# HeyWeCome/WhisprRec

Measured on AMD Instinct MI355X. Metric: BPR training triplets/sec, higher is better.
Workload: dtype f32; 1 GPU; BPRMF emb_size=64, synthetic 1000000 users x 1000000 items (uniform ids), batch 65536, SGD l2=0, plan build in timed region; batch=65536, emb_size=64, optimizer=SGD, plan_chunk_batches=64, tables=single GPU, step_stream=whisprrec_amd.hip_ops.PipelinedSgd, plan=group plan (no per-batch sort: flags + lists of the shared rows, wr_group.hip), chained_step_launch=True, plan_build=on a side stream, beside the steps of the chunk before

## Files before the change

### include/whisprrec_hip.h

```cpp
#ifndef WHISPRREC_HIP_H
#define WHISPRREC_HIP_H

#include <stdint.h>

#ifdef __cplusplus
extern "C" {
#endif

#define WR_ABI_VERSION 1

#define WR_OK 0
#define WR_E_NULL (-1)
#define WR_E_SHAPE (-2)
#define WR_E_WORKSPACE (-3)
#define WR_E_ALIGN (-4)
#define WR_E_RANGE (-5)

int32_t wr_abi_version(void);
const char *wr_last_error(void);
int32_t wr_device_info(int32_t *n_cu, int32_t *wave_size, char *arch, int32_t arch_len);

int64_t wr_bpr_fwd_workspace_bytes(int64_t B);
int32_t wr_bpr_fwd(const float *user_tab, int64_t n_users, const float *item_tab, int64_t n_items, int32_t D,
                   const int64_t *u, const int64_t *p, const int64_t *n, int64_t B, float *pos_score, float *neg_score,
                   float *coef, float *loss, void *workspace, int64_t workspace_bytes, void *stream);

int64_t wr_bprmf_plan_workspace_bytes(int64_t n_triplets, int64_t batch_size, int64_t n_users, int64_t n_items);
int32_t wr_bprmf_plan_build_i64(const int64_t *u, const int64_t *p, const int64_t *n, int64_t n_triplets,
                                int64_t batch_size, int64_t n_users, int64_t n_items, int32_t *tu, int32_t *tp,
                                int32_t *tn, int32_t *torig, int32_t *oc_item, int32_t *oc_src, int32_t *err_flag,
                                void *workspace, int64_t workspace_bytes, void *stream);
int32_t wr_bprmf_plan_build_i32(const int32_t *u, const int32_t *p, const int32_t *n, int64_t n_triplets,
                                int64_t batch_size, int64_t n_users, int64_t n_items, int32_t *tu, int32_t *tp,
                                int32_t *tn, int32_t *torig, int32_t *oc_item, int32_t *oc_src, int32_t *err_flag,
                                void *workspace, int64_t workspace_bytes, void *stream);

int64_t wr_bprmf_plan_small_max_batch(void);
int32_t wr_bprmf_plan_build_small_i64(const int64_t *u, const int64_t *p, const int64_t *n, int64_t n_triplets,
                                      int64_t batch_size, int64_t n_users, int64_t n_items, int32_t *tu, int32_t *tp,
                                      int32_t *tn, int32_t *torig, int32_t *oc_item, int32_t *oc_src, int32_t *err_flag,
                                      void *stream);
int32_t wr_bprmf_plan_build_small_i32(const int32_t *u, const int32_t *p, const int32_t *n, int64_t n_triplets,
                                      int64_t batch_size, int64_t n_users, int64_t n_items, int32_t *tu, int32_t *tp,
                                      int32_t *tn, int32_t *torig, int32_t *oc_item, int32_t *oc_src, int32_t *err_flag,
                                      void *stream);

int64_t wr_bprmf_plan_fast_workspace_bytes(int64_t n_triplets, int64_t batch_size, int64_t n_users, int64_t n_items);
int32_t wr_bprmf_plan_build_fast_i64(const int64_t *u, const int64_t *p, const int64_t *n, int64_t n_triplets,
                                     int64_t batch_size, int64_t n_users, int64_t n_items, int32_t *tu, int32_t *tp,
                                     int32_t *tn, int32_t *torig, int32_t *oc_item, int32_t *oc_src, int32_t *flags,
                                     void *workspace, int64_t workspace_bytes, void *stream);
int32_t wr_bprmf_plan_build_fast_i32(const int32_t *u, const int32_t *p, const int32_t *n, int64_t n_triplets,
                                     int64_t batch_size, int64_t n_users, int64_t n_items, int32_t *tu, int32_t *tp,
                                     int32_t *tn, int32_t *torig, int32_t *oc_item, int32_t *oc_src, int32_t *flags,
                                     void *workspace, int64_t workspace_bytes, void *stream);

int32_t wr_bprmf_plan_fast_marks_supported(int64_t n_triplets, int64_t batch_size, int64_t n_users, int64_t n_items);
int32_t wr_bprmf_plan_build_fast_marks_i64(const int64_t *u, const int64_t *p, const int64_t *n, int64_t n_triplets,
                                           int64_t batch_size, int64_t n_users, int64_t n_items, int32_t *tu, int32_t *tp,
                                           int32_t *tn, int32_t *torig, int32_t *oc_item, int32_t *oc_src, int32_t *flags,
                                           void *workspace, int64_t workspace_bytes, int32_t *bitmap, void *stream);
int32_t wr_bprmf_plan_build_fast_marks_i32(const int32_t *u, const int32_t *p, const int32_t *n, int64_t n_triplets,
                                           int64_t batch_size, int64_t n_users, int64_t n_items, int32_t *tu, int32_t *tp,
                                           int32_t *tn, int32_t *torig, int32_t *oc_item, int32_t *oc_src, int32_t *flags,
                                           void *workspace, int64_t workspace_bytes, int32_t *bitmap, void *stream);

typedef struct wr_bucket_side {
    int32_t n_buckets;
    const int32_t *row_bucket;
    const int32_t *bucket_start;
    const int32_t *bucket_rows;
    const int32_t *bucket_sub;
} wr_bucket_side;

int64_t wr_bprmf_plan_fast_mapped_workspace_bytes(int64_t n_triplets, int64_t batch_size, int64_t n_users, int64_t n_items,
                                                  int32_t n_buckets_users, int32_t n_buckets_items);
int32_t wr_bprmf_plan_build_fast_mapped_i64(const int64_t *u, const int64_t *p, const int64_t *n, int64_t n_triplets,
                                            int64_t batch_size, int64_t n_users, int64_t n_items,
                                            const wr_bucket_side *map_users, const wr_bucket_side *map_items, int32_t *tu,
                                            int32_t *tp, int32_t *tn, int32_t *torig, int32_t *oc_item, int32_t *oc_src,
                                            int32_t *flags, void *workspace, int64_t workspace_bytes, void *stream);
int32_t wr_bprmf_plan_build_fast_mapped_i32(const int32_t *u, const int32_t *p, const int32_t *n, int64_t n_triplets,
                                            int64_t batch_size, int64_t n_users, int64_t n_items,
                                            const wr_bucket_side *map_users, const wr_bucket_side *map_items, int32_t *tu,
                                            int32_t *tp, int32_t *tn, int32_t *torig, int32_t *oc_item, int32_t *oc_src,
                                            int32_t *flags, void *workspace, int64_t workspace_bytes, void *stream);

int32_t wr_sample_negatives_i64(const int64_t *users, int64_t n, int64_t n_users, int64_t n_items, const int64_t *clicked_ptr,
                                const int32_t *clicked_idx, uint64_t seed, uint64_t epoch, int64_t *neg_items,
                                int32_t *err_flag, void *stream);
int32_t wr_sample_negatives_i32(const int32_t *users, int64_t n, int64_t n_users, int64_t n_items, const int64_t *clicked_ptr,
                                const int32_t *clicked_idx, uint64_t seed, uint64_t epoch, int32_t *neg_items,
                                int32_t *err_flag, void *stream);

int32_t wr_epoch_prepare_range_i64(const int64_t *users, const int64_t *items, int64_t n, int64_t n_users, int64_t n_items,
                                   const int64_t *clicked_ptr, const int32_t *clicked_idx, uint64_t seed, uint64_t epoch,
                                   int64_t first, int64_t count, int64_t *out_users, int64_t *out_pos, int64_t *out_neg,
                                   int64_t *order_out, int32_t *err_flag, void *stream);
int32_t wr_epoch_prepare_range_i32(const int32_t *users, const int32_t *items, int64_t n, int64_t n_users, int64_t n_items,
                                   const int64_t *clicked_ptr, const int32_t *clicked_idx, uint64_t seed, uint64_t epoch,
                                   int64_t first, int64_t count, int32_t *out_users, int32_t *out_pos, int32_t *out_neg,
                                   int64_t *order_out, int32_t *err_flag, void *stream);

int64_t wr_pairset_capacity(int64_t n_pairs);
int32_t wr_pairset_build(const int64_t *clicked_ptr, const int32_t *clicked_idx, int64_t n_users, uint64_t *table,
                         int64_t capacity, int32_t *err_flag, void *stream);
int32_t wr_sample_negatives_set_i64(const int64_t *users, int64_t n, int64_t n_users, int64_t n_items, const uint64_t *pair_table,
                                    int64_t pair_capacity, uint64_t seed, uint64_t epoch, int64_t *neg_items,
                                    int32_t *err_flag, void *stream);
int32_t wr_sample_negatives_set_i32(const int32_t *users, int64_t n, int64_t n_users, int64_t n_items, const uint64_t *pair_table,
                                    int64_t pair_capacity, uint64_t seed, uint64_t epoch, int32_t *neg_items,
                                    int32_t *err_flag, void *stream);
int32_t wr_epoch_prepare_range_set_i64(const int64_t *users, const int64_t *items, int64_t n, int64_t n_users, int64_t n_items,
                                       const uint64_t *pair_table, int64_t pair_capacity, uint64_t seed, uint64_t epoch,
                                       int64_t first, int64_t count, int64_t *out_users, int64_t *out_pos, int64_t *out_neg,
                                       int64_t *order_out, int32_t *err_flag, void *stream);
int32_t wr_epoch_prepare_range_set_i32(const int32_t *users, const int32_t *items, int64_t n, int64_t n_users, int64_t n_items,
                                       const uint64_t *pair_table, int64_t pair_capacity, uint64_t seed, uint64_t epoch,
                                       int64_t first, int64_t count, int32_t *out_users, int32_t *out_pos, int32_t *out_neg,
                                       int64_t *order_out, int32_t *err_flag, void *stream);

int32_t wr_epoch_prepare_range_packed_i64(const uint64_t *packed_rows, int64_t n, int64_t n_users, int64_t n_items,
                                          const uint64_t *pair_table, int64_t pair_capacity, uint64_t seed, uint64_t epoch,
                                          int64_t first, int64_t count, int64_t *out_users, int64_t *out_pos, int64_t *out_neg,
                                          int64_t *order_out, int32_t *err_flag, void *stream);
int32_t wr_epoch_prepare_range_packed_i32(const uint64_t *packed_rows, int64_t n, int64_t n_users, int64_t n_items,
                                          const uint64_t *pair_table, int64_t pair_capacity, uint64_t seed, uint64_t epoch,
                                          int64_t first, int64_t count, int32_t *out_users, int32_t *out_pos, int32_t *out_neg,
                                          int64_t *order_out, int32_t *err_flag, void *stream);

int32_t wr_epoch_shuffle_i64(const int64_t *col0, const int64_t *col1, const int64_t *col2, int64_t n, uint64_t seed,
                             uint64_t epoch, int64_t *out0, int64_t *out1, int64_t *out2, int64_t *order_out, void *stream);
int32_t wr_epoch_shuffle_i32(const int32_t *col0, const int32_t *col1, const int32_t *col2, int64_t n, uint64_t seed,
                             uint64_t epoch, int32_t *out0, int32_t *out1, int32_t *out2, int64_t *order_out, void *stream);

typedef struct wr_hot_runs {
    const int32_t *piece_q, *piece_len, *run_q, *run_first, *run_np;
    const int32_t *u_piece_q, *u_piece_len, *u_run_q, *u_run_first, *u_run_np;
    const int32_t *counts_host;
    int64_t cap_pieces, cap_runs, cap_u_pieces, cap_u_runs;
} wr_hot_runs;
void wr_bprmf_hot_caps(int64_t batch_size, int32_t kind, int64_t *cap_pieces, int64_t *cap_runs);
int32_t wr_bprmf_plan_hot_runs(const int32_t *keys, int32_t kind, int64_t n_triplets, int64_t batch_size, int32_t *piece_q,
                               int32_t *piece_len, int32_t *run_q, int32_t *run_first, int32_t *run_np, int32_t *counts,
                               void *stream);

int64_t wr_bprmf_step_workspace_bytes(int64_t B, int32_t D);
int32_t wr_bprmf_step_sgd(float *user_tab, int64_t n_users, float *item_tab, int64_t n_items, int32_t D,
                          const int32_t *tu, const int32_t *tp, const int32_t *tn, const int32_t *oc_item,
                          const int32_t *oc_src, int64_t B, float lr, float l2, int32_t *stamp_u, int32_t *stamp_i,
                          int32_t step_id, float *loss_out, const wr_hot_runs *hot, void *workspace,
                          int64_t workspace_bytes, void *stream);

int32_t wr_bprmf_run_sgd(float *user_tab, int64_t n_users, float *item_tab, int64_t n_items, int32_t D,
                         const int32_t *tu, const int32_t *tp, const int32_t *tn, const int32_t *oc_item,
                         const int32_t *oc_src, int64_t n_triplets, int64_t batch_size, int64_t first_batch,
                         int64_t n_batches, float lr, float *loss_out, void *const *phase_events, const wr_hot_runs *hot,
                         void *workspace, int64_t workspace_bytes, void *stream);

int32_t wr_bprmf_chain_supported(const float *user_tab, const float *item_tab, int32_t D);
int64_t wr_bprmf_chain_sync_words(int64_t n_batches);
int32_t wr_bprmf_run_sgd_chain(float *user_tab, int64_t n_users, float *item_tab, int64_t n_items, int32_t D,
                               const int32_t *tu, const int32_t *tp, const int32_t *tn, const int32_t *oc_item,
                               const int32_t *oc_src, int64_t n_triplets, int64_t batch_size, int64_t first_batch,
                               int64_t n_batches, float lr, float *loss_out, const int32_t *tdef, const int32_t *def_q,
                               const int32_t *def_count_host, int64_t def_cap, int64_t def_limit, void *const *phase_events,
                               void *workspace, int64_t workspace_bytes, int32_t *sync, int64_t sync_words, void *stream);

int64_t wr_group_plan_words(int64_t n_triplets, int64_t batch_size, int64_t n_users, int64_t n_items);
int32_t wr_group_plan_layout(int64_t n_triplets, int64_t batch_size, int64_t n_users, int64_t n_items, int64_t *out);
int32_t wr_narrow_ids_i64(const int64_t *u, const int64_t *p, const int64_t *n, int32_t *u32, int32_t *p32, int32_t *n32,
                          int64_t count, void *stream);
int32_t wr_group_plan_build(const int32_t *u, const int32_t *p, const int32_t *n, int64_t n_triplets, int64_t batch_size,
                            int64_t n_users, int64_t n_items, int32_t *plan, int64_t plan_words, void *stream);
int64_t wr_bprmf_group_workspace_bytes(int64_t batch_size, int32_t D);
int64_t wr_bprmf_group_sync_words(int64_t n_batches);
int32_t wr_bprmf_group_supported(const float *user_tab, const float *item_tab, int32_t D);
int32_t wr_bprmf_run_sgd_group(float *user_tab, int64_t n_users, float *item_tab, int64_t n_items, int32_t D,
                               const int32_t *u, const int32_t *p, const int32_t *n, int64_t n_triplets, int64_t batch_size,
                               const int32_t *plan, int64_t plan_words, int64_t first_batch, int64_t n_batches, float lr,
                               float *loss_out, void *const *events, void *workspace, int64_t workspace_bytes, int32_t *sync,
                               int64_t sync_words, void *stream);

int32_t wr_bprmf_plan_overlap_marks(const int32_t *tu, const int32_t *tp, const int32_t *tn, int64_t n_triplets,
                                    int64_t batch_size, int64_t n_items, const int32_t *prev_bitmap, int32_t *bitmap,
                                    int32_t *tdef, int32_t *def_q, int64_t def_cap, int32_t *def_count, void *stream);

int32_t wr_bprmf_plan_overlap_deferred(const int32_t *tu, const int32_t *tp, const int32_t *tn, int64_t n_triplets,
                                       int64_t batch_size, int64_t n_items, const int32_t *prev_bitmap, const int32_t *bitmap,
                                       int32_t *tdef, int32_t *def_q, int64_t def_cap, int32_t *def_count, void *stream);

int32_t wr_bprmf_grads(const float *user_tab, int64_t n_users, const float *item_tab, int64_t n_items, int32_t D,
                       const int32_t *tu, const int32_t *tp, const int32_t *tn, const int32_t *oc_item,
                       const int32_t *oc_src, int64_t B, float *grad_u, float *grad_i, int32_t *stamp_u,
                       int32_t *stamp_i, int32_t step_id, float *loss_out, const wr_hot_runs *hot, void *workspace,
                       int64_t workspace_bytes, void *stream);

int32_t wr_sgd_decay_untouched(float *tab, int64_t n_rows, int32_t D, const int32_t *stamp, int32_t step_id, float lr,
                               float l2, void *stream);
int32_t wr_sgd_dense(float *tab, int64_t n_rows, int32_t D, const float *grad, const int32_t *stamp, int32_t step_id,
                     float lr, float l2, void *stream);
int32_t wr_adam_dense(float *tab, float *exp_avg, float *exp_avg_sq, int64_t n_rows, int32_t D, const float *grad,
                      const int32_t *stamp, int32_t step_id, int64_t adam_step, float lr, float l2, float beta1,
                      float beta2, float eps, void *stream);

int32_t wr_adam_dense_dev(float *tab, float *exp_avg, float *exp_avg_sq, int64_t n_rows, int32_t D, const float *grad,
                          const float *consts, int64_t n_consts, const int32_t *step_dev, float l2, float beta1, float beta2,
                          float eps, void *stream);

int32_t wr_adam_dense_dev_pair(float *tab_a, float *exp_avg_a, float *exp_avg_sq_a, int64_t n_rows_a, const float *grad_a,
                               float *tab_b, float *exp_avg_b, float *exp_avg_sq_b, int64_t n_rows_b, const float *grad_b,
                               int32_t D, const float *consts, int64_t n_consts, const int32_t *step_dev, float l2,
                               float beta1, float beta2, float eps, void *stream);
int32_t wr_counter_add(int32_t *counter, int32_t delta, void *stream);

int32_t wr_adam_consts(int64_t first_step, int64_t n_steps, float lr, float beta1, float beta2, float *consts_host);
int32_t wr_adam_rows_lazy(float *tab, float *exp_avg, float *exp_avg_sq, int32_t *last_step, int64_t n_rows, int32_t D,
                          const int32_t *keys, int64_t n_keys, const float *grad, int64_t adam_step, const float *consts,
                          int64_t n_consts, float l2, float beta1, float beta2, float eps, void *stream);
int32_t wr_adam_catchup_all(float *tab, float *exp_avg, float *exp_avg_sq, int32_t *last_step, int64_t n_rows, int32_t D,
                            int64_t adam_step, const float *consts, int64_t n_consts, float l2, float beta1, float beta2,
                            float eps, void *stream);
int32_t wr_sgd_rows_lazy(float *tab, int32_t *last_step, int64_t n_rows, int32_t D, const int32_t *keys, int64_t n_keys,
                         int64_t step, float lr, float l2, void *stream);
int32_t wr_sgd_catchup_all(float *tab, int32_t *last_step, int64_t n_rows, int32_t D, int64_t step, float lr, float l2,
                           void *stream);

int32_t wr_bprmf_step_adam(float *user_tab, int64_t n_users, float *item_tab, int64_t n_items, int32_t D, float *m_u,
                           float *v_u, float *m_i, float *v_i, int32_t *last_u, int32_t *last_i, const int32_t *tu,
                           const int32_t *tp, const int32_t *tn, const int32_t *oc_item, const int32_t *oc_src, int64_t B,
                           int64_t adam_step, float lr, float l2, float beta1, float beta2, float eps, float *loss_out,
                           const wr_hot_runs *hot, void *workspace, int64_t workspace_bytes, void *stream);
int32_t wr_bprmf_run_stateful(int32_t kind, float *user_tab, int64_t n_users, float *item_tab, int64_t n_items, int32_t D,
                              float *s1_u, float *s2_u, float *s1_i, float *s2_i, int32_t *last_u, int32_t *last_i,
                              const int32_t *tu, const int32_t *tp, const int32_t *tn, const int32_t *oc_item,
                              const int32_t *oc_src, int64_t n_triplets, int64_t batch_size, int64_t first_batch,
                              int64_t n_batches, int64_t step0, float lr, float rho, float eps, float *loss_out,
                              const wr_hot_runs *hot, void *workspace, int64_t workspace_bytes, void *stream);
int32_t wr_bprmf_step_adam_folded(float *user_tab, int64_t n_users, float *item_tab, int64_t n_items, int32_t D, float *m_u,
                                  float *v_u, float *m_i, float *v_i, int32_t *last_u, int32_t *last_i, const int32_t *tu,
                                  const int32_t *tp, const int32_t *tn, const int32_t *oc_item, const int32_t *oc_src,
                                  int64_t B, int64_t adam_step, float lr, const float *consts, int64_t n_consts, float l2,
                                  float beta1, float beta2, float eps, float *loss_out, void *workspace,
                                  int64_t workspace_bytes, void *stream);
int32_t wr_bprmf_run_adam_folded(float *user_tab, int64_t n_users, float *item_tab, int64_t n_items, int32_t D, float *m_u,
                                 float *v_u, float *m_i, float *v_i, int32_t *last_u, int32_t *last_i, const int32_t *tu,
                                 const int32_t *tp, const int32_t *tn, const int32_t *oc_item, const int32_t *oc_src,
                                 int64_t n_triplets, int64_t batch_size, int64_t first_batch, int64_t n_batches,
                                 int64_t adam_step0, float lr, const float *consts, int64_t n_consts, float l2, float beta1,
                                 float beta2, float eps, float *loss_out, const wr_hot_runs *hot, void *workspace,
                                 int64_t workspace_bytes, void *stream);
int32_t wr_bprmf_run_adam_folded_chain(float *user_tab, int64_t n_users, float *item_tab, int64_t n_items, int32_t D,
                                       float *m_u, float *v_u, float *m_i, float *v_i, int32_t *last_u, int32_t *last_i,
                                       const int32_t *tu, const int32_t *tp, const int32_t *tn, const int32_t *oc_item,
                                       const int32_t *oc_src, int64_t n_triplets, int64_t batch_size, int64_t first_batch,
                                       int64_t n_batches, int64_t adam_step0, float lr, const float *consts, int64_t n_consts,
                                       float l2, float beta1, float beta2, float eps, float *loss_out, const int32_t *tdef,
                                       const int32_t *def_q, const int32_t *def_count_host, int64_t def_cap, int64_t def_limit,
                                       void *workspace, int64_t workspace_bytes, int32_t *sync, int64_t sync_words,
                                       void *stream);
int32_t wr_bprmf_run_adam_lazy_bounded(float *user_tab, int64_t n_users, float *item_tab, int64_t n_items, int32_t D,
                                       float *m_u, float *v_u, float *m_i, float *v_i, int32_t *last_u, int32_t *last_i,
                                       const int32_t *tu, const int32_t *tp, const int32_t *tn, const int32_t *oc_item,
                                       const int32_t *oc_src, int64_t n_triplets, int64_t batch_size, int64_t first_batch,
                                       int64_t n_batches, int64_t adam_step0, float lr, const float *consts, int64_t n_consts,
                                       float l2, float beta1, float beta2, float eps, float *loss_out, const wr_hot_runs *hot,
                                       int64_t max_lag, int64_t *sweep_pos, void *workspace, int64_t workspace_bytes,
                                       void *stream);
int32_t wr_bprmf_run_sgd_lazy_bounded(float *user_tab, int64_t n_users, float *item_tab, int64_t n_items, int32_t D,
                                      int32_t *last_u, int32_t *last_i, int32_t *stamp_u, int32_t *stamp_i, int32_t step_id0,
                                      const int32_t *tu, const int32_t *tp, const int32_t *tn, const int32_t *oc_item,
                                      const int32_t *oc_src, int64_t n_triplets, int64_t batch_size, int64_t first_batch,
                                      int64_t n_batches, int64_t step0, float lr, float l2, float *loss_out,
                                      const wr_hot_runs *hot, int64_t max_lag, int64_t *sweep_pos, void *workspace,
                                      int64_t workspace_bytes, void *stream);
int32_t wr_bprmf_run_stateful_bounded(int32_t kind, float *user_tab, int64_t n_users, float *item_tab, int64_t n_items,
                                      int32_t D, float *s1_u, float *s2_u, float *s1_i, float *s2_i, int32_t *last_u,
                                      int32_t *last_i, const int32_t *tu, const int32_t *tp, const int32_t *tn,
                                      const int32_t *oc_item, const int32_t *oc_src, int64_t n_triplets, int64_t batch_size,
                                      int64_t first_batch, int64_t n_batches, int64_t step0, float lr, float rho, float eps,
                                      float *loss_out, const wr_hot_runs *hot, int64_t max_lag, int64_t *sweep_pos,
                                      void *workspace, int64_t workspace_bytes, void *stream);
int32_t wr_adadelta_decay_all(float *square_avg, float *acc_delta, int32_t *last_step, int64_t n_rows, int32_t D, int64_t step,
                              float rho, void *stream);
int32_t wr_bprmf_run_adam_lazy(float *user_tab, int64_t n_users, float *item_tab, int64_t n_items, int32_t D, float *m_u,
                               float *v_u, float *m_i, float *v_i, int32_t *last_u, int32_t *last_i, const int32_t *tu,
                               const int32_t *tp, const int32_t *tn, const int32_t *oc_item, const int32_t *oc_src,
                               int64_t n_triplets, int64_t batch_size, int64_t first_batch, int64_t n_batches,
                               int64_t adam_step0, float lr, const float *consts, int64_t n_consts, float l2, float beta1,
                               float beta2, float eps, float *loss_out, const wr_hot_runs *hot, void *workspace,
                               int64_t workspace_bytes, void *stream);
int32_t wr_bprmf_run_sgd_lazy(float *user_tab, int64_t n_users, float *item_tab, int64_t n_items, int32_t D, int32_t *last_u,
                              int32_t *last_i, int32_t *stamp_u, int32_t *stamp_i, int32_t step_id0, const int32_t *tu,
                              const int32_t *tp, const int32_t *tn, const int32_t *oc_item, const int32_t *oc_src,
                              int64_t n_triplets, int64_t batch_size, int64_t first_batch, int64_t n_batches, int64_t step0,
                              float lr, float l2, float *loss_out, const wr_hot_runs *hot, void *workspace,
                              int64_t workspace_bytes, void *stream);

int32_t wr_gather_rows(const float *tab, int64_t n_rows, int32_t D, const int64_t *idx, int64_t n, float *out,
                       void *stream);
int64_t wr_scatter_add_workspace_bytes(int64_t n, int64_t n_rows);
int32_t wr_scatter_add_rows(float *grad, int64_t n_rows, int32_t D, const int64_t *idx, const float *src, int64_t n,
                            int64_t padding_idx, float alpha, void *workspace, int64_t workspace_bytes, void *stream);

int64_t wr_scatter_plan_words(int64_t n_segments, int64_t seg_stride, int64_t n_rows);
int32_t wr_scatter_plan_build(const int64_t *idx, int64_t n_segments, int64_t seg_stride, const int32_t *seg_len, int64_t n_rows,
                              int64_t padding_idx, int32_t *plan, int64_t plan_words, void *stream);
int32_t wr_scatter_add_planned(float *table, int64_t n_rows, int32_t D, const int64_t *idx, int64_t n_segments,
                               int64_t seg_stride, int64_t segment, int64_t n, int64_t padding_idx, const float *src,
                               float alpha, const int32_t *plan, int64_t plan_words, void *stream);

int32_t wr_apply_rows_sorted(float *tab, int64_t n_rows, int32_t D, const int32_t *sorted_rows, const int32_t *perm,
                             const float *src, int64_t n, float alpha, void *stream);

int32_t wr_bprmf_shard_step(float *user_shard, int64_t n_user_rows, float *item_rows, int64_t n_rows, int64_t n_local_items,
                            int32_t D, const int32_t *tu, const int32_t *tp, const int32_t *tn, const int32_t *oc_item,
                            const int32_t *oc_src, int64_t B, int64_t global_batch, float lr, float *grad_slots,
                            float *loss_partial, const wr_hot_runs *hot, void *workspace, int64_t workspace_bytes,
                            void *stream);

int32_t wr_shard_route(const int32_t *u, const int32_t *p, const int32_t *n, int64_t n_triplets, int64_t batch_size, int32_t world,
                       int32_t rank, int64_t n_users, int64_t n_items, int64_t rows_per_owner, int64_t n_local_items,
                       int64_t list_cap, int32_t *vu, int32_t *vp, int32_t *vn, int32_t *send_rows, int32_t *send_cnt,
                       int32_t *err, void *stream);
int32_t wr_shard_pack(const int32_t *recv_rows, const int32_t *recv_cnt, int64_t n_batches, int32_t world, int64_t list_cap,
                      int64_t n_local_items, int64_t *serve_rows, int64_t serve_stride, int32_t *serve_off, int32_t *err,
                      void *stream);
int32_t wr_bprmf_shard_step_group(float *user_shard, int64_t n_user_rows, float *item_ext, int64_t n_ext_rows,
                                  int64_t n_local_items, int32_t D, const int32_t *vu, const int32_t *vp, const int32_t *vn,
                                  int64_t n_triplets, int64_t batch_size, const int32_t *plan, int64_t plan_words, int64_t batch,
                                  int64_t global_batch, float lr, float *grad_slots, float *loss_partial, void *workspace,
                                  int64_t workspace_bytes, int32_t *sync, int64_t sync_words, void *stream);

int32_t wr_spmm_csr(int64_t n_rows, const int64_t *row_ptr, const int32_t *col, const float *val, const float *X,
                    int32_t D, float *Y, float *acc, void *stream);
int32_t wr_spmm_csr_chunked(int64_t n_rows, int64_t n_chunks, const int64_t *chunk_ptr, const int32_t *chunk_row,
                            const int32_t *col, const float *val, const float *X, int32_t D, float *Y, float *acc,
                            float *partials, void *stream);

int64_t wr_spmm_dense_partials_bytes(int64_t n_tiles, int64_t K_pad, int64_t k_per_split, int32_t D);
typedef struct wr_dense_group {
    const float *A_T;
    const int32_t *cols;
    const int32_t *rows;
    float *partials;
    int64_t K_pad, k_per_split, n_tiles;
} wr_dense_group;
int32_t wr_spmm_dense_tiles(const wr_dense_group *unsplit, const wr_dense_group *split, const float *X, int64_t n_nodes,
                            int32_t D, float *Y, float *acc, void *stream);
int32_t wr_spmm_csr_chunked_modes(int64_t n_rows, int64_t n_chunks, const int64_t *chunk_ptr, const int32_t *chunk_row,
                                  const int32_t *col, const float *val, const float *X, int32_t D, float *Y, float *acc,
                                  float *partials, const int8_t *row_mode, void *stream);
int32_t wr_spmm_csr_chunked_levels(int64_t n_rows, int64_t n_chunks, const int64_t *chunk_ptr, const int32_t *chunk_row,
                                   const int32_t *col, const float *val, const float *X, int32_t D, float *Y, float *acc,
                                   float *partials, const int8_t *row_mode, int32_t levels, int32_t acc_from_x,
                                   float acc_scale, void *stream);

int32_t wr_spmm_fused_supported(int32_t D, const float *partials);
int32_t wr_spmm_csr_chunked_fused(int64_t n_rows, int64_t n_chunks, const int64_t *chunk_ptr, const int32_t *chunk_row,
                                  const int32_t *row_span, const int32_t *col, const float *val, const float *X, int32_t D,
                                  float *Y, float *acc, float *partials, const int8_t *row_mode, int32_t acc_from_x,
                                  float acc_scale, uint32_t *counters, void *stream);
int32_t wr_axpy(float *y, const float *x, int64_t numel, float alpha, int32_t overwrite, void *stream);
int32_t wr_embloss_sumsq(const float *user_tab, const float *item_tab, int32_t D, const int64_t *u, const int64_t *p,
                         const int64_t *n, int64_t B, float *sq3, void *workspace, int64_t workspace_bytes,
                         void *stream);

int32_t wr_rank_eval(const float *user_mat, int64_t n_user_rows, const float *item_tab, int64_t n_items, int32_t D,
                     const int64_t *eval_user, const int64_t *eval_target, int64_t n, const int64_t *mask_ptr,
                     const int32_t *mask_idx, int32_t *rank, float *target_score, void *stream);

int32_t wr_topk_supported(int32_t D, int32_t k);
int64_t wr_topk_workspace_bytes(int64_t n, int64_t n_items, int32_t D, int32_t k);
int32_t wr_topk_recommend(const float *user_mat, int64_t n_user_rows, const float *item_tab, int64_t n_items, int32_t D,
                          const int64_t *query_user, int64_t n, const int64_t *mask_ptr, const int32_t *mask_idx,
                          int32_t k, int32_t *out_item, float *out_score, void *workspace, int64_t workspace_bytes,
                          void *stream);

int64_t wr_lightgcn_loss_workspace_bytes(int64_t B);
int32_t wr_lightgcn_loss(const float *user_all, const float *item_all, const float *user_ego, const float *item_ego,
                         int64_t n_users, int64_t n_items, int32_t D, const int64_t *u, const int64_t *p, const int64_t *n,
                         int64_t B, float reg_weight, float *loss, float *sq3, void *workspace, int64_t workspace_bytes,
                         void *stream);
int32_t wr_embloss_grad(const float *user_tab, const float *item_tab, int32_t D, const int32_t *tu, const int32_t *oc_item,
                        const int32_t *oc_src, int64_t B, const float *sq3, float reg_weight, float *grad_user,
                        float *grad_item, void *stream);

int64_t wr_lightgcn_step_workspace_bytes(int64_t n_users, int64_t n_items, int32_t D, int64_t n_chunks, int64_t B);
int32_t wr_lightgcn_step(const float *user_tab, const float *item_tab, int64_t n_users, int64_t n_items, int32_t D,
                         int64_t n_chunks, const int64_t *chunk_ptr, const int32_t *chunk_row, const int32_t *col,
                         const float *val, int32_t levels, int32_t n_layers, const int64_t *u, const int64_t *p, const int64_t *n,
                         int64_t B, float reg_weight, int32_t trusted_indices, float *loss, float *grad, int32_t *err_flag,
                         void *workspace, int64_t workspace_bytes, void *stream);

#ifdef __cplusplus
}
#endif
#endif
```

### whisprrec_amd/abi.py

```python
import ctypes
import os

_HERE = os.path.dirname(os.path.abspath(__file__))
LIB_PATH = os.path.join(_HERE, "libwhisprrec_hip.so")

c_i32, c_i64, c_f32, c_vp = ctypes.c_int32, ctypes.c_int64, ctypes.c_float, ctypes.c_void_p

SIGNATURES = {
    "wr_abi_version": (c_i32, []),
    "wr_last_error": (ctypes.c_char_p, []),
    "wr_device_info": (c_i32, [c_vp, c_vp, c_vp, c_i32]),
    "wr_bpr_fwd_workspace_bytes": (c_i64, [c_i64]),
    "wr_bpr_fwd": (c_i32, [c_vp, c_i64, c_vp, c_i64, c_i32, c_vp, c_vp, c_vp, c_i64, c_vp, c_vp, c_vp, c_vp, c_vp, c_i64,
                           c_vp]),
    "wr_bprmf_plan_workspace_bytes": (c_i64, [c_i64, c_i64, c_i64, c_i64]),
    "wr_bprmf_plan_build_i64": (c_i32, [c_vp, c_vp, c_vp, c_i64, c_i64, c_i64, c_i64, c_vp, c_vp, c_vp, c_vp, c_vp, c_vp,
                                        c_vp, c_vp, c_i64, c_vp]),
    "wr_bprmf_plan_build_i32": (c_i32, [c_vp, c_vp, c_vp, c_i64, c_i64, c_i64, c_i64, c_vp, c_vp, c_vp, c_vp, c_vp, c_vp,
                                        c_vp, c_vp, c_i64, c_vp]),
    "wr_bprmf_plan_small_max_batch": (c_i64, []),
    "wr_bprmf_plan_build_small_i64": (c_i32, [c_vp, c_vp, c_vp, c_i64, c_i64, c_i64, c_i64, c_vp, c_vp, c_vp, c_vp, c_vp, c_vp,
                                              c_vp, c_vp]),
    "wr_bprmf_plan_build_small_i32": (c_i32, [c_vp, c_vp, c_vp, c_i64, c_i64, c_i64, c_i64, c_vp, c_vp, c_vp, c_vp, c_vp, c_vp,
                                              c_vp, c_vp]),
    "wr_bprmf_plan_fast_workspace_bytes": (c_i64, [c_i64, c_i64, c_i64, c_i64]),
    "wr_bprmf_plan_fast_mapped_workspace_bytes": (c_i64, [c_i64, c_i64, c_i64, c_i64, c_i32, c_i32]),
    "wr_bprmf_plan_build_fast_mapped_i64": (c_i32, [c_vp, c_vp, c_vp, c_i64, c_i64, c_i64, c_i64, c_vp, c_vp, c_vp, c_vp, c_vp,
                                                    c_vp, c_vp, c_vp, c_vp, c_vp, c_i64, c_vp]),
    "wr_bprmf_plan_build_fast_mapped_i32": (c_i32, [c_vp, c_vp, c_vp, c_i64, c_i64, c_i64, c_i64, c_vp, c_vp, c_vp, c_vp, c_vp,
                                                    c_vp, c_vp, c_vp, c_vp, c_vp, c_i64, c_vp]),
    "wr_bprmf_plan_build_fast_i64": (c_i32, [c_vp, c_vp, c_vp, c_i64, c_i64, c_i64, c_i64, c_vp, c_vp, c_vp, c_vp, c_vp,
                                             c_vp, c_vp, c_vp, c_i64, c_vp]),
    "wr_bprmf_plan_build_fast_i32": (c_i32, [c_vp, c_vp, c_vp, c_i64, c_i64, c_i64, c_i64, c_vp, c_vp, c_vp, c_vp, c_vp,
                                             c_vp, c_vp, c_vp, c_i64, c_vp]),
    "wr_sample_negatives_i64": (c_i32, [c_vp, c_i64, c_i64, c_i64, c_vp, c_vp, ctypes.c_uint64, ctypes.c_uint64, c_vp, c_vp,
                                        c_vp]),
    "wr_sample_negatives_i32": (c_i32, [c_vp, c_i64, c_i64, c_i64, c_vp, c_vp, ctypes.c_uint64, ctypes.c_uint64, c_vp, c_vp,
                                        c_vp]),
    "wr_epoch_prepare_range_i64": (c_i32, [c_vp, c_vp, c_i64, c_i64, c_i64, c_vp, c_vp, ctypes.c_uint64, ctypes.c_uint64, c_i64, c_i64,
                                           c_vp, c_vp, c_vp, c_vp, c_vp, c_vp]),
    "wr_epoch_prepare_range_i32": (c_i32, [c_vp, c_vp, c_i64, c_i64, c_i64, c_vp, c_vp, ctypes.c_uint64, ctypes.c_uint64, c_i64, c_i64,
                                           c_vp, c_vp, c_vp, c_vp, c_vp, c_vp]),
    "wr_pairset_capacity": (c_i64, [c_i64]),
    "wr_pairset_build": (c_i32, [c_vp, c_vp, c_i64, c_vp, c_i64, c_vp, c_vp]),
    "wr_sample_negatives_set_i64": (c_i32, [c_vp, c_i64, c_i64, c_i64, c_vp, c_i64, ctypes.c_uint64, ctypes.c_uint64, c_vp, c_vp,
                                            c_vp]),
    "wr_sample_negatives_set_i32": (c_i32, [c_vp, c_i64, c_i64, c_i64, c_vp, c_i64, ctypes.c_uint64, ctypes.c_uint64, c_vp, c_vp,
                                            c_vp]),
    "wr_epoch_prepare_range_set_i64": (c_i32, [c_vp, c_vp, c_i64, c_i64, c_i64, c_vp, c_i64, ctypes.c_uint64, ctypes.c_uint64, c_i64,
                                               c_i64, c_vp, c_vp, c_vp, c_vp, c_vp, c_vp]),
    "wr_epoch_prepare_range_set_i32": (c_i32, [c_vp, c_vp, c_i64, c_i64, c_i64, c_vp, c_i64, ctypes.c_uint64, ctypes.c_uint64, c_i64,
                                               c_i64, c_vp, c_vp, c_vp, c_vp, c_vp, c_vp]),
    "wr_epoch_prepare_range_packed_i64": (c_i32, [c_vp, c_i64, c_i64, c_i64, c_vp, c_i64, ctypes.c_uint64, ctypes.c_uint64, c_i64,
                                                  c_i64, c_vp, c_vp, c_vp, c_vp, c_vp, c_vp]),
    "wr_epoch_prepare_range_packed_i32": (c_i32, [c_vp, c_i64, c_i64, c_i64, c_vp, c_i64, ctypes.c_uint64, ctypes.c_uint64, c_i64,
                                                  c_i64, c_vp, c_vp, c_vp, c_vp, c_vp, c_vp]),
    "wr_epoch_shuffle_i64": (c_i32, [c_vp, c_vp, c_vp, c_i64, ctypes.c_uint64, ctypes.c_uint64, c_vp, c_vp, c_vp, c_vp, c_vp]),
    "wr_epoch_shuffle_i32": (c_i32, [c_vp, c_vp, c_vp, c_i64, ctypes.c_uint64, ctypes.c_uint64, c_vp, c_vp, c_vp, c_vp, c_vp]),
    "wr_bprmf_step_workspace_bytes": (c_i64, [c_i64, c_i32]),
    "wr_bprmf_hot_caps": (None, [c_i64, c_i32, c_vp, c_vp]),
    "wr_bprmf_plan_hot_runs": (c_i32, [c_vp, c_i32, c_i64, c_i64, c_vp, c_vp, c_vp, c_vp, c_vp, c_vp, c_vp]),
    "wr_bprmf_step_sgd": (c_i32, [c_vp, c_i64, c_vp, c_i64, c_i32, c_vp, c_vp, c_vp, c_vp, c_vp, c_i64, c_f32, c_f32,
                                  c_vp, c_vp, c_i32, c_vp, c_vp, c_vp, c_i64, c_vp]),
    "wr_bprmf_run_sgd": (c_i32, [c_vp, c_i64, c_vp, c_i64, c_i32, c_vp, c_vp, c_vp, c_vp, c_vp, c_i64, c_i64, c_i64,
                                 c_i64, c_f32, c_vp, c_vp, c_vp, c_vp, c_i64, c_vp]),
    "wr_bprmf_chain_supported": (c_i32, [c_vp, c_vp, c_i32]),
    "wr_bprmf_chain_sync_words": (c_i64, [c_i64]),
    "wr_bprmf_run_sgd_chain": (c_i32, [c_vp, c_i64, c_vp, c_i64, c_i32, c_vp, c_vp, c_vp, c_vp, c_vp, c_i64, c_i64, c_i64,
                                       c_i64, c_f32, c_vp, c_vp, c_vp, c_vp, c_i64, c_i64, c_vp, c_vp, c_i64, c_vp, c_i64,
                                       c_vp]),
    "wr_lightgcn_step_workspace_bytes": (c_i64, [c_i64, c_i64, c_i32, c_i64, c_i64]),
    "wr_lightgcn_step": (c_i32, [c_vp, c_vp, c_i64, c_i64, c_i32, c_i64, c_vp, c_vp, c_vp, c_vp, c_i32, c_i32, c_vp, c_vp, c_vp,
                                 c_i64, c_f32, c_i32, c_vp, c_vp, c_vp, c_vp, c_i64, c_vp]),
    "wr_shard_route": (c_i32, [c_vp, c_vp, c_vp, c_i64, c_i64, c_i32, c_i32, c_i64, c_i64, c_i64, c_i64, c_i64, c_vp, c_vp, c_vp,
                               c_vp, c_vp, c_vp, c_vp]),
    "wr_shard_pack": (c_i32, [c_vp, c_vp, c_i64, c_i32, c_i64, c_i64, c_vp, c_i64, c_vp, c_vp, c_vp]),
    "wr_bprmf_shard_step_group": (c_i32, [c_vp, c_i64, c_vp, c_i64, c_i64, c_i32, c_vp, c_vp, c_vp, c_i64, c_i64, c_vp, c_i64,
                                          c_i64, c_i64, c_f32, c_vp, c_vp, c_vp, c_i64, c_vp, c_i64, c_vp]),
    "wr_group_plan_words": (c_i64, [c_i64, c_i64, c_i64, c_i64]),
    "wr_group_plan_layout": (c_i32, [c_i64, c_i64, c_i64, c_i64, c_vp]),
    "wr_narrow_ids_i64": (c_i32, [c_vp, c_vp, c_vp, c_vp, c_vp, c_vp, c_i64, c_vp]),
    "wr_group_plan_build": (c_i32, [c_vp, c_vp, c_vp, c_i64, c_i64, c_i64, c_i64, c_vp, c_i64, c_vp]),
    "wr_bprmf_group_workspace_bytes": (c_i64, [c_i64, c_i32]),
    "wr_bprmf_group_sync_words": (c_i64, [c_i64]),
    "wr_bprmf_group_supported": (c_i32, [c_vp, c_vp, c_i32]),
    "wr_bprmf_run_sgd_group": (c_i32, [c_vp, c_i64, c_vp, c_i64, c_i32, c_vp, c_vp, c_vp, c_i64, c_i64, c_vp, c_i64, c_i64,
                                       c_i64, c_f32, c_vp, c_vp, c_vp, c_i64, c_vp, c_i64, c_vp]),
    "wr_bprmf_plan_overlap_deferred": (c_i32, [c_vp, c_vp, c_vp, c_i64, c_i64, c_i64, c_vp, c_vp, c_vp, c_vp, c_i64, c_vp,
                                               c_vp]),
    "wr_bprmf_plan_fast_marks_supported": (c_i32, [c_i64, c_i64, c_i64, c_i64]),
    "wr_bprmf_plan_build_fast_marks_i64": (c_i32, [c_vp, c_vp, c_vp, c_i64, c_i64, c_i64, c_i64, c_vp, c_vp, c_vp, c_vp, c_vp,
                                                   c_vp, c_vp, c_vp, c_i64, c_vp, c_vp]),
    "wr_bprmf_plan_build_fast_marks_i32": (c_i32, [c_vp, c_vp, c_vp, c_i64, c_i64, c_i64, c_i64, c_vp, c_vp, c_vp, c_vp, c_vp,
                                                   c_vp, c_vp, c_vp, c_i64, c_vp, c_vp]),
    "wr_bprmf_plan_overlap_marks": (c_i32, [c_vp, c_vp, c_vp, c_i64, c_i64, c_i64, c_vp, c_vp, c_vp, c_vp, c_i64, c_vp,
                                            c_vp]),
    "wr_bprmf_grads": (c_i32, [c_vp, c_i64, c_vp, c_i64, c_i32, c_vp, c_vp, c_vp, c_vp, c_vp, c_i64, c_vp, c_vp, c_vp,
                               c_vp, c_i32, c_vp, c_vp, c_vp, c_i64, c_vp]),
    "wr_sgd_decay_untouched": (c_i32, [c_vp, c_i64, c_i32, c_vp, c_i32, c_f32, c_f32, c_vp]),
    "wr_sgd_dense": (c_i32, [c_vp, c_i64, c_i32, c_vp, c_vp, c_i32, c_f32, c_f32, c_vp]),
    "wr_adam_dense": (c_i32, [c_vp, c_vp, c_vp, c_i64, c_i32, c_vp, c_vp, c_i32, c_i64, c_f32, c_f32, c_f32, c_f32,
                              c_f32, c_vp]),
    "wr_adam_dense_dev": (c_i32, [c_vp, c_vp, c_vp, c_i64, c_i32, c_vp, c_vp, c_i64, c_vp, c_f32, c_f32, c_f32, c_f32, c_vp]),
    "wr_adam_dense_dev_pair": (c_i32, [c_vp, c_vp, c_vp, c_i64, c_vp, c_vp, c_vp, c_vp, c_i64, c_vp, c_i32, c_vp, c_i64, c_vp,
                                       c_f32, c_f32, c_f32, c_f32, c_vp]),
    "wr_counter_add": (c_i32, [c_vp, c_i32, c_vp]),
    "wr_adam_consts": (c_i32, [c_i64, c_i64, c_f32, c_f32, c_f32, c_vp]),
    "wr_adam_rows_lazy": (c_i32, [c_vp, c_vp, c_vp, c_vp, c_i64, c_i32, c_vp, c_i64, c_vp, c_i64, c_vp, c_i64, c_f32, c_f32,
                                  c_f32, c_f32, c_vp]),
    "wr_adam_catchup_all": (c_i32, [c_vp, c_vp, c_vp, c_vp, c_i64, c_i32, c_i64, c_vp, c_i64, c_f32, c_f32, c_f32, c_f32,
                                    c_vp]),
    "wr_sgd_rows_lazy": (c_i32, [c_vp, c_vp, c_i64, c_i32, c_vp, c_i64, c_i64, c_f32, c_f32, c_vp]),
    "wr_sgd_catchup_all": (c_i32, [c_vp, c_vp, c_i64, c_i32, c_i64, c_f32, c_f32, c_vp]),
    "wr_bprmf_step_adam": (c_i32, [c_vp, c_i64, c_vp, c_i64, c_i32, c_vp, c_vp, c_vp, c_vp, c_vp, c_vp, c_vp, c_vp, c_vp, c_vp, c_vp,
                                   c_i64, c_i64, c_f32, c_f32, c_f32, c_f32, c_f32, c_vp, c_vp, c_vp, c_i64, c_vp]),
    "wr_bprmf_run_stateful": (c_i32, [c_i32, c_vp, c_i64, c_vp, c_i64, c_i32, c_vp, c_vp, c_vp, c_vp, c_vp, c_vp, c_vp, c_vp, c_vp,
                                      c_vp, c_vp, c_i64, c_i64, c_i64, c_i64, c_i64, c_f32, c_f32, c_f32, c_vp, c_vp, c_vp, c_i64,
                                      c_vp]),
    "wr_bprmf_step_adam_folded": (c_i32, [c_vp, c_i64, c_vp, c_i64, c_i32, c_vp, c_vp, c_vp, c_vp, c_vp, c_vp, c_vp, c_vp, c_vp, c_vp,
                                          c_vp, c_i64, c_i64, c_f32, c_vp, c_i64, c_f32, c_f32, c_f32, c_f32, c_vp, c_vp, c_i64,
                                          c_vp]),
    "wr_bprmf_run_adam_folded": (c_i32, [c_vp, c_i64, c_vp, c_i64, c_i32, c_vp, c_vp, c_vp, c_vp, c_vp, c_vp, c_vp, c_vp, c_vp, c_vp,
                                         c_vp, c_i64, c_i64, c_i64, c_i64, c_i64, c_f32, c_vp, c_i64, c_f32, c_f32, c_f32, c_f32,
                                         c_vp, c_vp, c_vp, c_i64, c_vp]),
    "wr_bprmf_run_adam_folded_chain": (c_i32, [c_vp, c_i64, c_vp, c_i64, c_i32, c_vp, c_vp, c_vp, c_vp, c_vp, c_vp, c_vp, c_vp, c_vp,
                                               c_vp, c_vp, c_i64, c_i64, c_i64, c_i64, c_i64, c_f32, c_vp, c_i64, c_f32, c_f32,
                                               c_f32, c_f32, c_vp, c_vp, c_vp, c_vp, c_i64, c_i64, c_vp, c_i64, c_vp, c_i64,
                                               c_vp]),
    "wr_bprmf_run_sgd_lazy_bounded": (c_i32, [c_vp, c_i64, c_vp, c_i64, c_i32, c_vp, c_vp, c_vp, c_vp, c_i32, c_vp, c_vp, c_vp,
                                              c_vp, c_vp, c_i64, c_i64, c_i64, c_i64, c_i64, c_f32, c_f32, c_vp, c_vp, c_i64,
                                              c_vp, c_vp, c_i64, c_vp]),
    "wr_bprmf_run_stateful_bounded": (c_i32, [c_i32, c_vp, c_i64, c_vp, c_i64, c_i32, c_vp, c_vp, c_vp, c_vp, c_vp, c_vp, c_vp,
                                              c_vp, c_vp, c_vp, c_vp, c_i64, c_i64, c_i64, c_i64, c_i64, c_f32, c_f32, c_f32,
                                              c_vp, c_vp, c_i64, c_vp, c_vp, c_i64, c_vp]),
    "wr_adadelta_decay_all": (c_i32, [c_vp, c_vp, c_vp, c_i64, c_i32, c_i64, c_f32, c_vp]),
    "wr_bprmf_run_adam_lazy_bounded": (c_i32, [c_vp, c_i64, c_vp, c_i64, c_i32, c_vp, c_vp, c_vp, c_vp, c_vp, c_vp, c_vp, c_vp,
                                               c_vp, c_vp, c_vp, c_i64, c_i64, c_i64, c_i64, c_i64, c_f32, c_vp, c_i64, c_f32,
                                               c_f32, c_f32, c_f32, c_vp, c_vp, c_i64, c_vp, c_vp, c_i64, c_vp]),
    "wr_bprmf_run_adam_lazy": (c_i32, [c_vp, c_i64, c_vp, c_i64, c_i32, c_vp, c_vp, c_vp, c_vp, c_vp, c_vp, c_vp, c_vp, c_vp, c_vp,
                                       c_vp, c_i64, c_i64, c_i64, c_i64, c_i64, c_f32, c_vp, c_i64, c_f32, c_f32, c_f32, c_f32,
                                       c_vp, c_vp, c_vp, c_i64, c_vp]),
    "wr_bprmf_run_sgd_lazy": (c_i32, [c_vp, c_i64, c_vp, c_i64, c_i32, c_vp, c_vp, c_vp, c_vp, c_i32, c_vp, c_vp, c_vp, c_vp, c_vp,
                                      c_i64, c_i64, c_i64, c_i64, c_i64, c_f32, c_f32, c_vp, c_vp, c_vp, c_i64, c_vp]),
    "wr_gather_rows": (c_i32, [c_vp, c_i64, c_i32, c_vp, c_i64, c_vp, c_vp]),
    "wr_scatter_add_workspace_bytes": (c_i64, [c_i64, c_i64]),
    "wr_scatter_add_rows": (c_i32, [c_vp, c_i64, c_i32, c_vp, c_vp, c_i64, c_i64, c_f32, c_vp, c_i64, c_vp]),
    "wr_scatter_plan_words": (c_i64, [c_i64, c_i64, c_i64]),
    "wr_scatter_plan_build": (c_i32, [c_vp, c_i64, c_i64, c_vp, c_i64, c_i64, c_vp, c_i64, c_vp]),
    "wr_scatter_add_planned": (c_i32, [c_vp, c_i64, c_i32, c_vp, c_i64, c_i64, c_i64, c_i64, c_i64, c_vp, c_f32, c_vp, c_i64,
                                       c_vp]),
    "wr_apply_rows_sorted": (c_i32, [c_vp, c_i64, c_i32, c_vp, c_vp, c_vp, c_i64, c_f32, c_vp]),
    "wr_bprmf_shard_step": (c_i32, [c_vp, c_i64, c_vp, c_i64, c_i64, c_i32, c_vp, c_vp, c_vp, c_vp, c_vp, c_i64, c_i64, c_f32,
                                    c_vp, c_vp, c_vp, c_vp, c_i64, c_vp]),
    "wr_spmm_csr": (c_i32, [c_i64, c_vp, c_vp, c_vp, c_vp, c_i32, c_vp, c_vp, c_vp]),
    "wr_spmm_csr_chunked": (c_i32, [c_i64, c_i64, c_vp, c_vp, c_vp, c_vp, c_vp, c_i32, c_vp, c_vp, c_vp, c_vp]),
    "wr_spmm_dense_partials_bytes": (c_i64, [c_i64, c_i64, c_i64, c_i32]),
    "wr_spmm_dense_tiles": (c_i32, [c_vp, c_vp, c_vp, c_i64, c_i32, c_vp, c_vp, c_vp]),
    "wr_spmm_csr_chunked_levels": (c_i32, [c_i64, c_i64, c_vp, c_vp, c_vp, c_vp, c_vp, c_i32, c_vp, c_vp, c_vp, c_vp, c_i32,
                                           c_i32, c_f32, c_vp]),
    "wr_spmm_fused_supported": (c_i32, [c_i32, c_vp]),
    "wr_spmm_csr_chunked_fused": (c_i32, [c_i64, c_i64, c_vp, c_vp, c_vp, c_vp, c_vp, c_vp, c_i32, c_vp, c_vp, c_vp, c_vp, c_i32,
                                          c_f32, c_vp, c_vp]),
    "wr_spmm_csr_chunked_modes": (c_i32, [c_i64, c_i64, c_vp, c_vp, c_vp, c_vp, c_vp, c_i32, c_vp, c_vp, c_vp, c_vp, c_vp]),
    "wr_axpy": (c_i32, [c_vp, c_vp, c_i64, c_f32, c_i32, c_vp]),
    "wr_rank_eval": (c_i32, [c_vp, c_i64, c_vp, c_i64, c_i32, c_vp, c_vp, c_i64, c_vp, c_vp, c_vp, c_vp, c_vp]),
    "wr_topk_supported": (c_i32, [c_i32, c_i32]),
    "wr_topk_workspace_bytes": (c_i64, [c_i64, c_i64, c_i32, c_i32]),
    "wr_topk_recommend": (c_i32, [c_vp, c_i64, c_vp, c_i64, c_i32, c_vp, c_i64, c_vp, c_vp, c_i32, c_vp, c_vp, c_vp, c_i64,
                                  c_vp]),
    "wr_lightgcn_loss_workspace_bytes": (c_i64, [c_i64]),
    "wr_lightgcn_loss": (c_i32, [c_vp, c_vp, c_vp, c_vp, c_i64, c_i64, c_i32, c_vp, c_vp, c_vp, c_i64, c_f32, c_vp, c_vp, c_vp,
                                 c_i64, c_vp]),
    "wr_embloss_grad": (c_i32, [c_vp, c_vp, c_i32, c_vp, c_vp, c_vp, c_i64, c_vp, c_f32, c_vp, c_vp, c_vp]),
    "wr_embloss_sumsq": (c_i32, [c_vp, c_vp, c_i32, c_vp, c_vp, c_vp, c_i64, c_vp, c_vp, c_i64, c_vp]),
}



class HotRuns(ctypes.Structure):
    _fields_ = [("piece_q", c_vp), ("piece_len", c_vp), ("run_q", c_vp), ("run_first", c_vp), ("run_np", c_vp),
                ("u_piece_q", c_vp), ("u_piece_len", c_vp), ("u_run_q", c_vp), ("u_run_first", c_vp), ("u_run_np", c_vp),
                ("counts_host", c_vp), ("cap_pieces", c_i64), ("cap_runs", c_i64), ("cap_u_pieces", c_i64),
                ("cap_u_runs", c_i64)]


class DenseGroup(ctypes.Structure):
    _fields_ = [("A_T", c_vp), ("cols", c_vp), ("rows", c_vp), ("partials", c_vp), ("K_pad", c_i64), ("k_per_split", c_i64),
                ("n_tiles", c_i64)]


class BucketSide(ctypes.Structure):
    _fields_ = [("n_buckets", c_i32), ("row_bucket", c_vp), ("bucket_start", c_vp), ("bucket_rows", c_vp), ("bucket_sub", c_vp)]


_lib = None


class WhisprRecHipError(RuntimeError):
    pass


def lib():
    global _lib
    if _lib is None:
        if not os.path.exists(LIB_PATH):
            raise WhisprRecHipError(
                "libwhisprrec_hip.so is missing at %s — build it with `python -c 'import __graft_entry__ as g; g.build()'` "
                "or `make -C whisprrec_amd/csrc`.  There is no CPU fallback." % LIB_PATH)
        import torch
        handle = ctypes.CDLL(LIB_PATH)
        for name, (res, args) in SIGNATURES.items():
            fn = getattr(handle, name)
            fn.restype = res
            fn.argtypes = args
        if handle.wr_abi_version() != 1:
            raise WhisprRecHipError("ABI version mismatch: library %d, binding 1" % handle.wr_abi_version())
        _lib = handle
    return _lib


def last_error():
    return lib().wr_last_error().decode("utf-8", "replace")


def check(rc, what):
    if rc != 0:
        raise WhisprRecHipError("%s failed (rc=%d): %s" % (what, rc, last_error()))


def check_size(nbytes, what):
    if nbytes < 0:
        raise WhisprRecHipError("%s failed (rc=%d): %s" % (what, nbytes, last_error()))
    return int(nbytes)
```

### whisprrec_amd/csrc/wr_group.hip

```cpp
#include "wr_common.h"
#include <hip/hip_ext.h>

#include <algorithm>

namespace wr {

constexpr int kGpThreads = 1024;
constexpr unsigned kGpRangeBits = 18;
constexpr int kGpWords = 1 << (kGpRangeBits - 5);
constexpr int kGpCap = 8192;
constexpr int kGpBins = 4096;
constexpr int kGpMaxBin = 256;
constexpr int kGpMaxRanges = 8;
constexpr int64_t kGpMaxBatch = 1 << 17;
constexpr int kGpLongRun = 64;
constexpr int kGpMetaWords = 16;
#ifndef WR_GP_DBG
#define WR_GP_DBG 0
#endif

struct GroupLayout {
    int64_t nb, B, fw;
    int R_u, R_i, cap_u, cap_i;
    unsigned mask_u, mask_i, hbits_u, hbits_i;
    int64_t flags, ucnt, icnt, ul_row, ul_src, il_row, il_src, total;
    int64_t zero_words;
};

static inline int ranges_for(int64_t n_rows, unsigned *mask, unsigned *hbits, int *cap) {
    unsigned bits = kGpRangeBits;
    while (bits < kGpRangeBits + 3 && (int64_t(1) << bits) < n_rows) ++bits;
    *mask = (1u << bits) - 1u;
    *hbits = bits;
    const int R = 1 << (bits - kGpRangeBits);
    *cap = kGpCap;
    return R;
}

static bool group_layout(int64_t n, int64_t B, int64_t n_users, int64_t n_items, GroupLayout &L) {
    if (n <= 0 || n >= (int64_t(1) << 31) || B <= 0 || B > kGpMaxBatch) return false;
    if (n_users <= 0 || n_users >= (int64_t(1) << 31) || n_items <= 0 || n_items >= (int64_t(1) << 31)) return false;
    L.nb = (n + B - 1) / B;
    L.B = B;
    L.fw = (B + 31) / 32;
    L.R_u = ranges_for(n_users, &L.mask_u, &L.hbits_u, &L.cap_u);
    L.R_i = ranges_for(n_items, &L.mask_i, &L.hbits_i, &L.cap_i);
    L.flags = kGpMetaWords;
    L.ucnt = L.flags + L.nb * L.fw * 4;
    L.icnt = L.ucnt + align_up(L.nb * L.R_u, 4);
    L.zero_words = L.icnt + align_up(L.nb * L.R_i, 4);
    L.ul_row = L.zero_words;
    L.ul_src = L.ul_row + L.nb * L.R_u * (int64_t)L.cap_u;
    L.il_row = L.ul_src + L.nb * L.R_u * (int64_t)L.cap_u;
    L.il_src = L.il_row + L.nb * L.R_i * (int64_t)L.cap_i;
    L.total = L.il_src + L.nb * L.R_i * (int64_t)L.cap_i;
    return true;
}

struct GpDev {
    int *meta;
    unsigned *flags;
    int *ucnt, *icnt;
    int *ul_row, *ul_src, *il_row, *il_src;
    int R_u, R_i, cap_u, cap_i;
    unsigned mask_u, mask_i, hbits_u, hbits_i;
    int fw;
};

static inline GpDev group_dev(int32_t *plan, const GroupLayout &L) {
    return GpDev{plan, reinterpret_cast<unsigned *>(plan + L.flags), plan + L.ucnt, plan + L.icnt, plan + L.ul_row,
                 plan + L.ul_src, plan + L.il_row, plan + L.il_src, L.R_u, L.R_i, L.cap_u, L.cap_i, L.mask_u, L.mask_i,
                 L.hbits_u, L.hbits_i, (int)L.fw};
}

template <typename F>
__device__ __forceinline__ void gp_scan(const int *__restrict__ a, int cnt, F f) {
    if ((reinterpret_cast<uintptr_t>(a) & 15u) == 0) {
        const int n4 = cnt >> 2;
        const int4 *a4 = reinterpret_cast<const int4 *>(a);
        int i = threadIdx.x;
        for (; i + 3 * kGpThreads < n4; i += 4 * kGpThreads) {
            int4 v[4];
#pragma unroll
            for (int q = 0; q < 4; ++q) v[q] = a4[i + q * kGpThreads];
#pragma unroll
            for (int q = 0; q < 4; ++q) {
                const int at = 4 * (i + q * kGpThreads);
                f(v[q].x, at);
                f(v[q].y, at + 1);
                f(v[q].z, at + 2);
                f(v[q].w, at + 3);
            }
        }
        for (; i < n4; i += kGpThreads) {
            const int4 v = a4[i];
            f(v.x, 4 * i);
            f(v.y, 4 * i + 1);
            f(v.z, 4 * i + 2);
            f(v.w, 4 * i + 3);
        }
        for (int j = (n4 << 2) + threadIdx.x; j < cnt; j += kGpThreads) f(a[j], j);
    } else {
        for (int j = threadIdx.x; j < cnt; j += kGpThreads) f(a[j], j);
    }
}

__global__ __launch_bounds__(kGpThreads) void group_plan_kernel(const int *__restrict__ u, const int *__restrict__ p,
                                                                 const int *__restrict__ n, int64_t n_total, int B, int nb,
                                                                 int n_users, int n_items, GpDev L) {
    extern __shared__ __attribute__((aligned(16))) unsigned gp_lds[];
    unsigned *seen = gp_lds;
    unsigned long long *keys = reinterpret_cast<unsigned long long *>(gp_lds);
    unsigned *multi = gp_lds + 2 * kGpCap;
    unsigned *f0 = multi + kGpWords, *f1 = f0 + L.fw, *f2 = f1 + L.fw;
    int &n_list = *reinterpret_cast<int *>(f2 + L.fw);
    const int per = L.R_u + L.R_i;
    const unsigned lb = xcd_contiguous_id(blockIdx.x, gridDim.x);
    const int b = (int)(lb / (unsigned)per), rr = (int)(lb % (unsigned)per);
    const bool item = rr >= L.R_u;
    const unsigned r = (unsigned)(item ? rr - L.R_u : rr);
    const int64_t base = (int64_t)b * B;
    const int Bb = (int)((base + B <= n_total) ? B : (n_total - base));
    const unsigned n_rows = (unsigned)(item ? n_items : n_users);
    const unsigned mask = item ? L.mask_i : L.mask_u;
    const unsigned rb = (item ? L.hbits_i : L.hbits_u) - kGpRangeBits, rsel = (1u << rb) - 1u;
    for (int i = threadIdx.x; i < kGpWords; i += kGpThreads) {
        seen[i] = 0u;
        multi[i] = 0u;
    }
    for (int i = threadIdx.x; i < 3 * L.fw; i += kGpThreads) f0[i] = 0u;
    if (threadIdx.x == 0) n_list = 0;
    __syncthreads();
    auto mark = [&](int row, int) {
        if ((unsigned)row >= n_rows) {
            L.meta[0] = 1;
            return;
        }
        const unsigned h = (unsigned)row & mask;
        if ((h & rsel) != r) return;
        const unsigned bit = h >> rb, m = 1u << (bit & 31u);
        const unsigned old = atomicOr(&seen[bit >> 5], m);
        if (old & m) atomicOr(&multi[bit >> 5], m);
    };
    if (!(WR_GP_DBG & 8)) {
        if (item) {
            gp_scan(p + base, Bb, mark);
            gp_scan(n + base, Bb, mark);
        } else {
            gp_scan(u + base, Bb, mark);
        }
    }
    __syncthreads();
    auto several = [&](int row) -> bool {
        const unsigned h = (unsigned)row & mask;
        if ((h & rsel) != r) return false;
        const unsigned bit = h >> rb;
        return (multi[bit >> 5] >> (bit & 31u)) & 1u;
    };
    auto append = [&](int row, unsigned src) {
        const int pos = atomicAdd(&n_list, 1);
        if (pos < kGpCap) keys[pos] = ((unsigned long long)(unsigned)row << 32) | src;
    };
    if (!(WR_GP_DBG & 2)) {
        const bool next = b + 1 < nb && !(WR_GP_DBG & 16);
        const int64_t nbase = base + B;
        const int Bn = next ? (int)((nbase + B <= n_total) ? B : (n_total - nbase)) : 0;
        auto defer = [&](int row, int t) {
            if (several(row)) atomicOr(&f2[t >> 5], 1u << (t & 31));
        };
        if (item) {
            gp_scan(p + base, Bb, [&](int row, int t) {
                if (several(row)) {
                    atomicOr(&f0[t >> 5], 1u << (t & 31));
                    append(row, (unsigned)t << 1);
                }
            });
            gp_scan(n + base, Bb, [&](int row, int t) {
                if (several(row)) {
                    atomicOr(&f1[t >> 5], 1u << (t & 31));
                    append(row, ((unsigned)t << 1) | 1u);
                }
            });
            gp_scan(p + nbase, Bn, defer);
            gp_scan(n + nbase, Bn, defer);
        } else {
            gp_scan(u + base, Bb, [&](int row, int t) {
                if (several(row)) {
                    atomicOr(&f0[t >> 5], 1u << (t & 31));
                    append(row, (unsigned)t << 1);
                }
            });
            gp_scan(u + nbase, Bn, defer);
        }
    }
    __syncthreads();
    if (!(WR_GP_DBG & 4)) {
        unsigned *fb = L.flags + (int64_t)b * L.fw * 4;
        for (int w = threadIdx.x; w < L.fw; w += kGpThreads) {
            if (f0[w]) __hip_atomic_fetch_or(fb + 4 * w + (item ? 1 : 0), f0[w], __ATOMIC_RELAXED, __HIP_MEMORY_SCOPE_AGENT);
            if (item && f1[w]) __hip_atomic_fetch_or(fb + 4 * w + 2, f1[w], __ATOMIC_RELAXED, __HIP_MEMORY_SCOPE_AGENT);
            if (f2[w])
                __hip_atomic_fetch_or(fb + 4 * (L.fw + w) + 3, f2[w], __ATOMIC_RELAXED, __HIP_MEMORY_SCOPE_AGENT);
        }
    }
    const int cap = item ? L.cap_i : L.cap_u, R = item ? L.R_i : L.R_u;
    int m = n_list;
    if (m > cap) {
        if (threadIdx.x == 0) L.meta[1] = 1;
        m = cap;
    }
    int *cnt = reinterpret_cast<int *>(multi);
    unsigned short *out16 = reinterpret_cast<unsigned short *>(multi + kGpBins);
    int *wave_tot = reinterpret_cast<int *>(f0);
    auto bin_of = [&](unsigned long long k) -> int { return (int)(((((unsigned)(k >> 32)) & mask) >> rb) & (kGpBins - 1)); };
    int *lrow = (item ? L.il_row : L.ul_row) + ((int64_t)b * R + r) * cap, *lsrc = (item ? L.il_src : L.ul_src) + ((int64_t)b * R + r) * cap;
    __syncthreads();
    for (int i = threadIdx.x; i < kGpBins; i += kGpThreads) cnt[i] = 0;
    __syncthreads();
    if (!(WR_GP_DBG & 1)) {
        for (int j = threadIdx.x; j < m; j += kGpThreads) atomicAdd(&cnt[bin_of(keys[j])], 1);
        __syncthreads();
        constexpr int kOwn = kGpBins / kGpThreads;
        const int c0 = (int)threadIdx.x * kOwn;
        int local = 0;
#pragma unroll
        for (int j = 0; j < kOwn; ++j) local += cnt[c0 + j];
        int incl = local;
#pragma unroll
        for (int d = 1; d < 64; d <<= 1) {
            const int v = __shfl_up(incl, d, 64);
            if ((int)(threadIdx.x & 63) >= d) incl += v;
        }
        if ((threadIdx.x & 63) == 63) wave_tot[threadIdx.x >> 6] = incl;
        __syncthreads();
        int run = incl - local;
        for (int w = 0; w < (int)(threadIdx.x >> 6); ++w) run += wave_tot[w];
#pragma unroll
        for (int j = 0; j < kOwn; ++j) {
            const int c = cnt[c0 + j];
            cnt[c0 + j] = run;
            run += c;
        }
        __syncthreads();
        for (int j = threadIdx.x; j < m; j += kGpThreads) out16[atomicAdd(&cnt[bin_of(keys[j])], 1)] = (unsigned short)j;
        __syncthreads();
        for (int j = threadIdx.x; j < m; j += kGpThreads) {
            const unsigned long long k = keys[j];
            const int bin = bin_of(k);
            const int lo = bin ? cnt[bin - 1] : 0, hi = cnt[bin];
            if (hi - lo > kGpMaxBin) {
                L.meta[1] = 1;
                continue;
            }
            int pos = lo, same = 0;
            for (int jj = lo; jj < hi; ++jj) {
                const unsigned long long o = keys[out16[jj]];
                pos += o < k ? 1 : 0;
                same += (unsigned)(o >> 32) == (unsigned)(k >> 32) ? 1 : 0;
            }
            if (same > kGpLongRun) L.meta[2] = 1;
            lrow[pos] = (int)(k >> 32);
            lsrc[pos] = (int)(unsigned)k;
        }
    } else {
        for (int j = threadIdx.x; j < m; j += kGpThreads) {
            lrow[j] = (int)(keys[j] >> 32);
            lsrc[j] = (int)(unsigned)keys[j];
        }
    }
    if (threadIdx.x == 0) (item ? L.icnt : L.ucnt)[(int64_t)b * R + r] = m;
}

__global__ __launch_bounds__(kBlock) void narrow_ids_kernel(const int64_t *__restrict__ u, const int64_t *__restrict__ p,
                                                             const int64_t *__restrict__ n, int *__restrict__ u32,
                                                             int *__restrict__ p32, int *__restrict__ n32, int64_t cnt) {
    const int64_t i = (int64_t)blockIdx.x * kBlock + threadIdx.x;
    if (i >= cnt) return;
    const int64_t a = u[i], b = p[i], c = n[i];
    u32[i] = (a >= 0 && a < (int64_t(1) << 31)) ? (int)a : -1;
    p32[i] = (b >= 0 && b < (int64_t(1) << 31)) ? (int)b : -1;
    n32[i] = (c >= 0 && c < (int64_t(1) << 31)) ? (int)c : -1;
}

constexpr int kGsTile = 32;
constexpr int kGsAhead = 8;
constexpr int kGsShards = 64;
constexpr int kGsShardStride = 16;
constexpr int kGsStepWords = kGsShards * kGsShardStride;
constexpr int kGsDefChunk = 32;
constexpr int kGsLdsInts = 1024 + 8;
constexpr unsigned kGsSpinLimit = 1u << 22;

struct GsBatch {
    const int *u, *p, *n;
    const uint4 *flags;
    const int *ul_row, *ul_src, *ul_cnt, *il_row, *il_src, *il_cnt;
    int B, R_u, R_i, cap_u, cap_i;
};

struct GsArgs {
    float *U, *I;
    int D;
    float lr;
    GsBatch cur;
    float *Z, *ZU, *partials;
    float denom;
    GsBatch prev;
    const float *Zp, *ZUp, *partials_prev;
    int n_partials_prev;
    float denom_prev;
    float *loss_prev;
    int nA, nIT, nUT, nDS, tiles_at, side_at;
    int chained;
    unsigned *done, *timeout;
    float *Gs;
    int nL;
};

template <int NV>
__device__ __forceinline__ Row<NV> row_zero() {
    Row<NV> r;
#pragma unroll
    for (int k = 0; k < NV; ++k) r.v[k] = make_float4(0.f, 0.f, 0.f, 0.f);
    return r;
}

template <int T, int NV, bool FULL>
__device__ __forceinline__ void gs_single(const GsArgs &a, int t, int u, int p, int n, bool us, bool ps, bool ns, int lane,
                                          float &terms) {
    const Row<NV> ur = load_row<T, NV, FULL>(a.U, u, a.D, lane);
    const Row<NV> pr = load_row<T, NV, FULL>(a.I, p, a.D, lane);
    const Row<NV> nr = load_row<T, NV, FULL>(a.I, n, a.D, lane);
    const float sp = team_sum<T>(dot_partial<NV>(ur, pr));
    const float sn = team_sum<T>(dot_partial<NV>(ur, nr));
    float term, c;
    bpr_terms(sp, sn, a.denom, term, c);
    terms += term;
    Row<NV> g, z;
#pragma unroll
    for (int k = 0; k < NV; ++k) {
        g.v[k] = make_float4(c * (pr.v[k].x - nr.v[k].x), c * (pr.v[k].y - nr.v[k].y), c * (pr.v[k].z - nr.v[k].z),
                             c * (pr.v[k].w - nr.v[k].w));
        z.v[k] = make_float4(c * ur.v[k].x, c * ur.v[k].y, c * ur.v[k].z, c * ur.v[k].w);
    }
    const float lr = a.lr;
    if (!us) {
        Row<NV> w;
#pragma unroll
        for (int k = 0; k < NV; ++k)
            w.v[k] = make_float4(ur.v[k].x - lr * g.v[k].x, ur.v[k].y - lr * g.v[k].y, ur.v[k].z - lr * g.v[k].z,
                                 ur.v[k].w - lr * g.v[k].w);
        store_row<T, NV, FULL>(a.U, u, a.D, lane, w);
    } else {
        store_row<T, NV, FULL>(a.ZU, t, a.D, lane, g);
    }
    if (!ps) {
        if (a.Gs != nullptr && p >= a.nL) {
            store_row<T, NV, FULL>(a.Gs, p - a.nL, a.D, lane, z);
        } else {
            Row<NV> w;
#pragma unroll
            for (int k = 0; k < NV; ++k)
                w.v[k] = make_float4(pr.v[k].x - lr * z.v[k].x, pr.v[k].y - lr * z.v[k].y, pr.v[k].z - lr * z.v[k].z,
                                     pr.v[k].w - lr * z.v[k].w);
            store_row<T, NV, FULL>(a.I, p, a.D, lane, w);
        }
    }
    if (!ns) {
        if (a.Gs != nullptr && n >= a.nL) {
            Row<NV> zn;
#pragma unroll
            for (int k = 0; k < NV; ++k) zn.v[k] = make_float4(-z.v[k].x, -z.v[k].y, -z.v[k].z, -z.v[k].w);
            store_row<T, NV, FULL>(a.Gs, n - a.nL, a.D, lane, zn);
        } else {
            Row<NV> w;
#pragma unroll
            for (int k = 0; k < NV; ++k)
                w.v[k] = make_float4(nr.v[k].x - lr * (-z.v[k].x), nr.v[k].y - lr * (-z.v[k].y), nr.v[k].z - lr * (-z.v[k].z),
                                     nr.v[k].w - lr * (-z.v[k].w));
            store_row<T, NV, FULL>(a.I, n, a.D, lane, w);
        }
    }
    if (ps || ns) store_row<T, NV, FULL>(a.Z, t, a.D, lane, z);
}

__device__ __forceinline__ void gs_wait_tiles(const GsArgs &a) {
    if (threadIdx.x < 64) {
        const int j = (int)threadIdx.x;
        const int n_sig = a.nIT + a.nUT;
        const unsigned want = j < kGsShards ? (unsigned)((n_sig - j + kGsShards - 1) / kGsShards) : 0u;
        const unsigned *shard = a.done + (j < kGsShards ? j : 0) * kGsShardStride;
        unsigned spins = 0;
        for (;;) {
            const bool ok = __hip_atomic_load(shard, __ATOMIC_RELAXED, __HIP_MEMORY_SCOPE_AGENT) >= want;
            if (__all(ok)) break;
            __builtin_amdgcn_s_sleep(8);
            if (++spins > kGsSpinLimit) {
                if (j == 0) __hip_atomic_store(a.timeout, 1u, __ATOMIC_RELAXED, __HIP_MEMORY_SCOPE_AGENT);
                break;
            }
        }
        __builtin_amdgcn_fence(__ATOMIC_ACQUIRE, "agent");
        asm volatile("s_waitcnt vmcnt(0)" ::: "memory");
    }
    __syncthreads();
}

__device__ __forceinline__ bool gs_tile_of(const int *__restrict__ cnt, int R, int cap, int q, int &seg, int &e0, int &len) {
    int c[kGpMaxRanges];
#pragma unroll
    for (int s = 0; s < kGpMaxRanges; ++s) c[s] = cnt[s < R ? s : 0];
    asm volatile("" : "+v"(c[0]), "+v"(c[1]), "+v"(c[2]), "+v"(c[3]), "+v"(c[4]), "+v"(c[5]), "+v"(c[6]), "+v"(c[7]));
#pragma unroll
    for (int s = 0; s < kGpMaxRanges; ++s)
        if (s >= R) c[s] = 0;
    bool found = false;
#pragma unroll
    for (int s = 0; s < kGpMaxRanges; ++s) {
        const int cs = min(c[s], cap);
        const int nt = (cs + kGsTile - 1) / kGsTile;
        if (!found && q < nt) {
            seg = s;
            e0 = q * kGsTile;
            len = cs;
            found = true;
        }
        if (!found) q -= nt;
    }
    return found;
}

struct GsTile {
    const int *lrow, *lsrc;
    int e0, len;
    int er, es, before;
};

__device__ __forceinline__ void gs_tile_fetch(GsTile &tl, const int *__restrict__ l_row, const int *__restrict__ l_src, int seg,
                                              int cap, int e0, int len, int B) {
    tl.lrow = l_row + (int64_t)seg * cap;
    tl.lsrc = l_src + (int64_t)seg * cap;
    tl.e0 = e0;
    tl.len = len;
    tl.er = -1;
    tl.es = 0;
    tl.before = -1;
    const int e = e0 + (int)threadIdx.x;
    if (threadIdx.x < kGsTile + kGsAhead && e < len) {
        tl.er = tl.lrow[e];
        tl.es = tl.lsrc[e];
    }
    if (threadIdx.x == 0 && e0 > 0) tl.before = tl.lrow[e0 - 1];
}

template <int T, int NV, bool FULL, bool WT>
__device__ __forceinline__ void gs_tile_finish(float *__restrict__ W, int D, float lr, int B, const float *__restrict__ Z,
                                               const GsTile &tl, int *__restrict__ lds, float *__restrict__ Gs = nullptr,
                                               int nL = 0) {
    int *rows_t = lds, *src_t = rows_t + (kGsTile + kGsAhead), *heads = src_t + (kGsTile + kGsAhead);
    int &n_heads = heads[kGsTile];
    constexpr int TEAMS = kBlock / T;
    const int lane = threadIdx.x % T;
    __syncthreads();
    if (threadIdx.x == 0) n_heads = 0;
    if (threadIdx.x < kGsTile + kGsAhead) {
        rows_t[threadIdx.x] = tl.er;
        src_t[threadIdx.x] = min(max(tl.es, 0), 2 * B - 1);
    }
    __syncthreads();
    if (threadIdx.x < kGsTile) {
        const int r = rows_t[threadIdx.x];
        const int bf = threadIdx.x == 0 ? tl.before : rows_t[threadIdx.x - 1];
        if (r >= 0 && bf != r) heads[atomicAdd(&n_heads, 1)] = threadIdx.x;
    }
    __syncthreads();
    const int nh = n_heads;
    for (int h = threadIdx.x / T; h < nh; h += TEAMS) {
        const int j0 = heads[h];
        const int r = rows_t[j0];
        const bool slot = Gs != nullptr && r >= nL;
        Row<NV> ir = row_zero<NV>();
        if (!slot) ir = load_row<T, NV, FULL>(W, r, D, lane);
        const int s0 = src_t[j0];
        const bool two = rows_t[j0 + 1] == r;
        const int s1 = src_t[j0 + 1];
        const Row<NV> z0 = load_row<T, NV, FULL>(Z, s0 >> 1, D, lane);
        Row<NV> z1 = row_zero<NV>();
        if (two) z1 = load_row<T, NV, FULL>(Z, s1 >> 1, D, lane);
        Row<NV> g;
        const float g0 = (s0 & 1) ? -1.0f : 1.0f, g1 = (s1 & 1) ? -1.0f : 1.0f;
#pragma unroll
        for (int k = 0; k < NV; ++k) {
            g.v[k].x = fmaf(g0, z0.v[k].x, 0.f);
            g.v[k].y = fmaf(g0, z0.v[k].y, 0.f);
            g.v[k].z = fmaf(g0, z0.v[k].z, 0.f);
            g.v[k].w = fmaf(g0, z0.v[k].w, 0.f);
        }
        if (two) {
#pragma unroll
            for (int k = 0; k < NV; ++k) {
                g.v[k].x = fmaf(g1, z1.v[k].x, g.v[k].x);
                g.v[k].y = fmaf(g1, z1.v[k].y, g.v[k].y);
                g.v[k].z = fmaf(g1, z1.v[k].z, g.v[k].z);
                g.v[k].w = fmaf(g1, z1.v[k].w, g.v[k].w);
            }
            auto add_z = [&](int src) {
                const Row<NV> z = load_row<T, NV, FULL>(Z, src >> 1, D, lane);
                const float sgn = (src & 1) ? -1.0f : 1.0f;
#pragma unroll
                for (int k = 0; k < NV; ++k) {
                    g.v[k].x = fmaf(sgn, z.v[k].x, g.v[k].x);
                    g.v[k].y = fmaf(sgn, z.v[k].y, g.v[k].y);
                    g.v[k].z = fmaf(sgn, z.v[k].z, g.v[k].z);
                    g.v[k].w = fmaf(sgn, z.v[k].w, g.v[k].w);
                }
            };
            int j = j0 + 2;
            for (; j < kGsTile + kGsAhead && rows_t[j] == r; ++j) add_z(src_t[j]);
            if (j == kGsTile + kGsAhead)
                for (int e = tl.e0 + j; e < tl.len && tl.lrow[e] == r; ++e) add_z(min(max(tl.lsrc[e], 0), 2 * B - 1));
        }
        if (slot) {
            store_row<T, NV, FULL>(Gs, r - nL, D, lane, g);
            continue;
        }
        Row<NV> wv;
#pragma unroll
        for (int k = 0; k < NV; ++k)
            wv.v[k] = make_float4(ir.v[k].x - lr * g.v[k].x, ir.v[k].y - lr * g.v[k].y, ir.v[k].z - lr * g.v[k].z,
                                  ir.v[k].w - lr * g.v[k].w);
        if constexpr (WT) store_row_wt<T, NV, FULL>(W, r, D, lane, wv);
        else store_row<T, NV, FULL>(W, r, D, lane, wv);
    }
}

#ifndef WR_GS_WAVES
#define WR_GS_WAVES 8
#endif
#ifndef WR_GS_DBG
#define WR_GS_DBG 0
#endif

template <int T, int NV, bool FULL, bool WT>
__device__ __forceinline__ void gs_list_tiles(float *__restrict__ W, int D, float lr, const int *__restrict__ l_row,
                                              const int *__restrict__ l_src, const int *__restrict__ l_cnt, int R, int cap,
                                              int B, const float *__restrict__ Z, int w, int nw, int *__restrict__ lds,
                                              float *__restrict__ Gs = nullptr, int nL = 0) {
    for (int q = w;; q += nw) {
        int seg, e0, len;
        if (!gs_tile_of(l_cnt, R, cap, q, seg, e0, len)) break;
        GsTile tl;
        gs_tile_fetch(tl, l_row, l_src, seg, cap, e0, len, B);
        gs_tile_finish<T, NV, FULL, WT>(W, D, lr, B, Z, tl, lds, Gs, nL);
    }
}

template <int T, int NV, bool FULL>
__global__ __launch_bounds__(kBlock, NV == 1 ? WR_GS_WAVES : 1) void bprmf_group_step(GsArgs a) {
    __shared__ float scratch[kBlock / 64];
    __shared__ __attribute__((aligned(16))) int lds[kGsLdsInts];
    constexpr int TEAMS = kBlock / T;
    const int lane = threadIdx.x % T;
    int b = (int)blockIdx.x;
    if (b >= a.tiles_at && b < a.tiles_at + a.nIT + a.nUT) {
        const int w = b - a.tiles_at;
        const bool wt = a.nA > 0;
        if (!(WR_GS_DBG & 1)) {
            if (w < a.nIT) {
                if (wt) gs_list_tiles<T, NV, FULL, true>(a.I, a.D, a.lr, a.prev.il_row, a.prev.il_src, a.prev.il_cnt, a.prev.R_i, a.prev.cap_i,
                                                         a.prev.B, a.Zp, w, a.nIT, lds, a.Gs, a.nL);
                else gs_list_tiles<T, NV, FULL, false>(a.I, a.D, a.lr, a.prev.il_row, a.prev.il_src, a.prev.il_cnt, a.prev.R_i, a.prev.cap_i,
                                                       a.prev.B, a.Zp, w, a.nIT, lds, a.Gs, a.nL);
            } else {
                if (wt) gs_list_tiles<T, NV, FULL, true>(a.U, a.D, a.lr, a.prev.ul_row, a.prev.ul_src, a.prev.ul_cnt, a.prev.R_u, a.prev.cap_u,
                                                         a.prev.B, a.ZUp, w - a.nIT, a.nUT, lds);
                else gs_list_tiles<T, NV, FULL, false>(a.U, a.D, a.lr, a.prev.ul_row, a.prev.ul_src, a.prev.ul_cnt, a.prev.R_u, a.prev.cap_u,
                                                       a.prev.B, a.ZUp, w - a.nIT, a.nUT, lds);
            }
        }
        if (wt) {
            asm volatile("s_waitcnt vmcnt(0)" ::: "memory");
            __syncthreads();
            if (threadIdx.x == 0)
                __hip_atomic_fetch_add(a.done + (w % kGsShards) * kGsShardStride, 1u, __ATOMIC_RELAXED, __HIP_MEMORY_SCOPE_AGENT);
        }
        if (w == 0 && a.loss_prev != nullptr) {
            const float s0 = strided_partial_sum(a.partials_prev, a.n_partials_prev);
            const float s = block_sum(s0, scratch);
            if (threadIdx.x == 0) a.loss_prev[0] = s / a.denom_prev;
        }
        return;
    }
    if (b >= a.tiles_at) b -= a.nIT + a.nUT;
    float terms = 0.f;
    int slot;
    if (b >= a.side_at && b < a.side_at + a.nDS) {
        const int w = b - a.side_at;
        int *dl = lds, &total_s = lds[kGsDefChunk * 32];
        const int fw = (a.cur.B + 31) / 32;
        const int per = (fw + a.nDS - 1) / a.nDS;
        const int w_end = min(fw, (w + 1) * per);
        bool waited = false;
        for (int c0 = w * per; c0 < w_end; c0 += kGsDefChunk) {
            const int wi = c0 + (int)threadIdx.x;
            unsigned m = 0u, us = 0u, ps = 0u, ns = 0u;
            if (threadIdx.x < kGsDefChunk && wi < w_end) {
                const uint4 f = a.cur.flags[wi];
                m = f.w;
                us = f.x;
                ps = f.y;
                ns = f.z;
            }
            int cnt = __popc(m), incl = cnt;
#pragma unroll
            for (int d = 1; d < 64; d <<= 1) {
                const int v = __shfl_up(incl, d, 64);
                if ((int)(threadIdx.x & 63) >= d) incl += v;
            }
            if (threadIdx.x == 63) total_s = incl;
            int at = incl - cnt;
            while (m) {
                const int bit = __ffs(m) - 1;
                m &= m - 1;
                dl[at++] = ((wi * 32 + bit) << 3) | (((us >> bit) & 1u) ? 4 : 0) | (((ps >> bit) & 1u) ? 1 : 0) |
                           (((ns >> bit) & 1u) ? 2 : 0);
            }
            __syncthreads();
            const int total = (WR_GS_DBG & 2) ? 0 : total_s;
            const int e0 = (int)threadIdx.x / T, e1 = e0 + TEAMS;
            int t0 = 0, u0 = 0, p0 = 0, n0 = 0, t1 = 0, u1 = 0, p1 = 0, n1 = 0;
            if (e0 < total) {
                t0 = min(dl[e0] >> 3, a.cur.B - 1);
                u0 = a.cur.u[t0];
                p0 = a.cur.p[t0];
                n0 = a.cur.n[t0];
            }
            if (e1 < total) {
                t1 = min(dl[e1] >> 3, a.cur.B - 1);
                u1 = a.cur.u[t1];
                p1 = a.cur.p[t1];
                n1 = a.cur.n[t1];
            }
            if (!waited) {
                if (!(WR_GS_DBG & 4)) gs_wait_tiles(a);
                waited = true;
            }
            if (e0 < total) gs_single<T, NV, FULL>(a, t0, u0, p0, n0, dl[e0] & 4, dl[e0] & 1, dl[e0] & 2, lane, terms);
            if (e1 < total) gs_single<T, NV, FULL>(a, t1, u1, p1, n1, dl[e1] & 4, dl[e1] & 1, dl[e1] & 2, lane, terms);
            for (int e = e1 + TEAMS; e < total; e += TEAMS) {
                const int t = min(dl[e] >> 3, a.cur.B - 1);
                gs_single<T, NV, FULL>(a, t, a.cur.u[t], a.cur.p[t], a.cur.n[t], dl[e] & 4, dl[e] & 1, dl[e] & 2, lane, terms);
            }
            __syncthreads();
        }
        slot = a.nA + w;
    } else {
        if (b >= a.side_at) b -= a.nDS;
        const int t = b * TEAMS + (int)threadIdx.x / T;
        const int tc = min(t, a.cur.B - 1);
        uint4 f = a.cur.flags[tc >> 5];
        int u = a.cur.u[tc], p = a.cur.p[tc], n = a.cur.n[tc];
#if WR_GS_DBG & 8
        f = make_uint4(0u, 0u, 0u, 0u);
#endif
        asm volatile("" : "+v"(u), "+v"(p), "+v"(n), "+v"(f.x), "+v"(f.y), "+v"(f.z), "+v"(f.w));
        const unsigned bit = 1u << (t & 31);
        if (t < a.cur.B && !(a.chained && (f.w & bit)))
            gs_single<T, NV, FULL>(a, t, u, p, n, f.x & bit, f.y & bit, f.z & bit, lane, terms);
        slot = b;
    }
    if (lane != 0) terms = 0.f;
    const float sum = block_sum(terms, scratch);
    if (threadIdx.x == 0) a.partials[slot] = sum;
}

static inline int gs_teams_per_block(int D) { return D >= 64 ? kBlock / 16 : (D == 32 ? kBlock / 8 : (D == 16 ? kBlock / 4 : (D == 8 ? kBlock / 2 : (D == 4 ? kBlock : kBlock / 16)))); }

static inline int64_t gs_ws_one(int64_t B, int32_t D) {
    const int64_t nA = (B + gs_teams_per_block(D) - 1) / gs_teams_per_block(D);
    return 2 * align_up(B * (int64_t)D * 4, 256) + align_up((nA + 512) * 4, 256);
}

static inline bool gs_shape_ok(const float *U, const float *I, int32_t D) {
    return (D * 4) % 128 == 0 && (reinterpret_cast<uintptr_t>(U) & 127u) == 0 && (reinterpret_cast<uintptr_t>(I) & 127u) == 0;
}

#ifndef WR_GS_TILES_AT
#define WR_GS_TILES_AT 0
#endif
#ifndef WR_GS_SIDE_AT
#define WR_GS_SIDE_AT 12
#endif
#ifndef WR_GS_NUT
#define WR_GS_NUT 256
#endif
#ifndef WR_GS_NDS
#define WR_GS_NDS 64
#endif
#ifndef WR_GS_NIT
#define WR_GS_NIT 1024
#endif

template <int T, int NV, bool FULL>
static int32_t launch_group_steps(float *U, float *I, int32_t D, const int32_t *u, const int32_t *p, const int32_t *n,
                                  int64_t n_triplets, const GroupLayout &L, const GpDev &G, int64_t first_batch,
                                  int64_t n_batches, float lr, float *loss_out, void *workspace, uint32_t *sync,
                                  int64_t sync_words, hipStream_t stream, void *const *events, int n_cu,
                                  float *grad_slots = nullptr, int64_t n_local_items = 0, int64_t global_batch = 0) {
    const int64_t B = L.B;
    const int64_t ws_one = gs_ws_one(B, D), zb = align_up(B * (int64_t)D * 4, 256);
    char *ws = reinterpret_cast<char *>(workspace);
    float *Zs[2] = {reinterpret_cast<float *>(ws), reinterpret_cast<float *>(ws + ws_one)};
    float *ZUs[2] = {reinterpret_cast<float *>(ws + zb), reinterpret_cast<float *>(ws + ws_one + zb)};
    float *Ps[2] = {reinterpret_cast<float *>(ws + 2 * zb), reinterpret_cast<float *>(ws + ws_one + 2 * zb)};
    constexpr int TEAMS = kBlock / T;
    WR_HIP(hipMemsetAsync(sync, 0, (size_t)(n_batches * kGsStepWords) * 4, stream));
    uint32_t *timeout = sync + (sync_words - 4);
    int nDS = WR_GS_NDS;
    while (nDS > n_cu / 4 && nDS > 1) nDS >>= 1;
    auto batch_of = [&](int64_t b) {
        const int64_t off = b * B;
        const int Bk = (int)((off + B <= n_triplets) ? B : (n_triplets - off));
        return GsBatch{u + off, p + off, n + off, reinterpret_cast<const uint4 *>(G.flags + b * L.fw * 4),
                       G.ul_row + b * L.R_u * (int64_t)L.cap_u, G.ul_src + b * L.R_u * (int64_t)L.cap_u, G.ucnt + b * L.R_u,
                       G.il_row + b * L.R_i * (int64_t)L.cap_i, G.il_src + b * L.R_i * (int64_t)L.cap_i, G.icnt + b * L.R_i,
                       Bk, L.R_u, L.R_i, L.cap_u, L.cap_i};
    };
    auto ev = [&](int64_t k, int j) { return events ? reinterpret_cast<hipEvent_t>(events[2 * k + j]) : (hipEvent_t) nullptr; };
    int n_partials_prev = 0;
    for (int64_t k = 0; k <= n_batches; ++k) {
        GsArgs a{};
        a.U = U;
        a.I = I;
        a.D = D;
        a.lr = lr;
        a.done = sync + (k < n_batches ? k : 0) * kGsStepWords;
        a.timeout = timeout;
        a.Gs = grad_slots;
        a.nL = (int)n_local_items;
        const bool have_cur = k < n_batches, have_prev = k > 0;
        if (have_cur) {
            a.cur = batch_of(first_batch + k);
            a.Z = Zs[k & 1];
            a.ZU = ZUs[k & 1];
            a.partials = Ps[k & 1];
            a.denom = global_batch > 0 ? (float)global_batch : (float)a.cur.B;
            a.nA = (int)((a.cur.B + TEAMS - 1) / TEAMS);
            a.nDS = have_prev ? nDS : 0;
            a.chained = have_prev ? 1 : 0;
        }
        if (have_prev) {
            a.prev = batch_of(first_batch + k - 1);
            a.Zp = Zs[(k - 1) & 1];
            a.ZUp = ZUs[(k - 1) & 1];
            a.partials_prev = Ps[(k - 1) & 1];
            a.n_partials_prev = n_partials_prev;
            a.denom_prev = global_batch > 0 ? (float)global_batch : (float)a.prev.B;
            a.loss_prev = loss_out ? loss_out + (k - 1) : nullptr;
            a.nIT = (int)std::min<int64_t>(WR_GS_NIT, (2 * B + kGsTile - 1) / kGsTile + L.R_i);
            a.nUT = (int)std::min<int64_t>(WR_GS_NUT, (B + kGsTile - 1) / kGsTile + L.R_u);
        }
        a.tiles_at = (int)((int64_t)a.nA * WR_GS_TILES_AT / 16);
        a.side_at = std::max(a.tiles_at, (int)((int64_t)a.nA * WR_GS_SIDE_AT / 16));
        const dim3 grid((unsigned)(a.nA + a.nIT + a.nUT + a.nDS));
        hipEvent_t e0 = have_cur ? ev(k, 0) : nullptr, e1 = have_cur ? ev(k, 1) : nullptr;
        if (e0 != nullptr || e1 != nullptr)
            hipExtLaunchKernelGGL((bprmf_group_step<T, NV, FULL>), grid, dim3(kBlock), 0, stream, e0, e1, 0, a);
        else
            hipLaunchKernelGGL((bprmf_group_step<T, NV, FULL>), grid, dim3(kBlock), 0, stream, a);
        WR_LAUNCH_CHECK("bprmf_group_step");
        n_partials_prev = a.nA + a.nDS;
    }
    return WR_OK;
}

}

using namespace wr;

extern "C" {

int64_t wr_group_plan_words(int64_t n_triplets, int64_t batch_size, int64_t n_users, int64_t n_items) {
    GroupLayout L;
    if (!group_layout(n_triplets, batch_size, n_users, n_items, L)) return 0;
    return L.total;
}

int32_t wr_group_plan_layout(int64_t n_triplets, int64_t batch_size, int64_t n_users, int64_t n_items, int64_t *out) {
    WR_REQUIRE(out != nullptr, WR_E_NULL, "out is NULL");
    GroupLayout L;
    WR_REQUIRE(group_layout(n_triplets, batch_size, n_users, n_items, L), WR_E_RANGE,
               "group plan not applicable to n=%lld, batch=%lld", (long long)n_triplets, (long long)batch_size);
    const int64_t v[16] = {L.nb, L.fw, L.R_u, L.R_i, (int64_t)L.mask_u, (int64_t)L.mask_i, L.flags, L.ucnt, L.icnt, L.ul_row,
                           L.ul_src, L.il_row, L.il_src, L.total, L.cap_u, L.cap_i};
    for (int i = 0; i < 16; ++i) out[i] = v[i];
    return WR_OK;
}

int32_t wr_narrow_ids_i64(const int64_t *u, const int64_t *p, const int64_t *n, int32_t *u32, int32_t *p32, int32_t *n32,
                          int64_t count, void *stream_) {
    WR_REQUIRE(u && p && n && u32 && p32 && n32, WR_E_NULL, "index arrays must not be NULL");
    WR_REQUIRE(count >= 0 && count < (int64_t(1) << 40), WR_E_SHAPE, "count out of range");
    if (count == 0) return WR_OK;
    hipLaunchKernelGGL(narrow_ids_kernel, dim3((unsigned)((count + kBlock - 1) / kBlock)), dim3(kBlock), 0,
                       reinterpret_cast<hipStream_t>(stream_), u, p, n, u32, p32, n32, count);
    WR_LAUNCH_CHECK("narrow_ids_kernel");
    return WR_OK;
}

int32_t wr_group_plan_build(const int32_t *u, const int32_t *p, const int32_t *n, int64_t n_triplets, int64_t batch_size,
                            int64_t n_users, int64_t n_items, int32_t *plan, int64_t plan_words, void *stream_) {
    WR_REQUIRE(u && p && n && plan, WR_E_NULL, "index arrays / plan must not be NULL");
    GroupLayout L;
    WR_REQUIRE(group_layout(n_triplets, batch_size, n_users, n_items, L), WR_E_RANGE,
               "group plan not applicable to n=%lld, batch=%lld", (long long)n_triplets, (long long)batch_size);
    WR_REQUIRE(aligned16(plan) && plan_words >= L.total, WR_E_WORKSPACE, "group plan: %lld words < %lld", (long long)plan_words,
               (long long)L.total);
    WR_REQUIRE(L.nb * (L.R_u + L.R_i) < (int64_t(1) << 31), WR_E_SHAPE, "group plan: too many batches in one plan");
    hipStream_t stream = reinterpret_cast<hipStream_t>(stream_);
    WR_HIP(hipMemsetAsync(plan, 0, (size_t)L.zero_words * 4, stream));
    const size_t lds = (size_t)(2 * kGpCap + kGpWords + 3 * L.fw + 4) * 4;
    static bool attr_set = false;
    if (!attr_set) {
        WR_HIP(hipFuncSetAttribute(reinterpret_cast<const void *>(group_plan_kernel), hipFuncAttributeMaxDynamicSharedMemorySize,
                                   (int)((2 * kGpCap + kGpWords + 3 * ((kGpMaxBatch + 31) / 32) + 4) * 4)));
        attr_set = true;
    }
    const GpDev G = group_dev(plan, L);
    hipLaunchKernelGGL(group_plan_kernel, dim3((unsigned)(L.nb * (L.R_u + L.R_i))), dim3(kGpThreads), lds, stream, u, p, n,
                       n_triplets, (int)batch_size, (int)L.nb, (int)n_users, (int)n_items, G);
    WR_LAUNCH_CHECK("group_plan_kernel");
    return WR_OK;
}

int64_t wr_bprmf_group_workspace_bytes(int64_t batch_size, int32_t D) { return 2 * gs_ws_one(batch_size, D); }

int64_t wr_bprmf_group_sync_words(int64_t n_batches) { return n_batches < 0 ? WR_E_SHAPE : (n_batches + 1) * kGsStepWords + 4; }

int32_t wr_bprmf_group_supported(const float *user_tab, const float *item_tab, int32_t D) {
    return (user_tab && item_tab && D >= 4 && D <= 1024 && D % 4 == 0 && gs_shape_ok(user_tab, item_tab, D)) ? 1 : 0;
}

int32_t wr_bprmf_run_sgd_group(float *user_tab, int64_t n_users, float *item_tab, int64_t n_items, int32_t D,
                               const int32_t *u, const int32_t *p, const int32_t *n, int64_t n_triplets, int64_t batch_size,
                               const int32_t *plan, int64_t plan_words, int64_t first_batch, int64_t n_batches, float lr,
                               float *loss_out, void *const *events, void *workspace, int64_t workspace_bytes, int32_t *sync,
                               int64_t sync_words, void *stream_) {
    int32_t rc;
    if ((rc = check_table(user_tab, n_users, D, "user_tab")) != WR_OK) return rc;
    if ((rc = check_table(item_tab, n_items, D, "item_tab")) != WR_OK) return rc;
    WR_REQUIRE(u && p && n && plan && sync, WR_E_NULL, "index arrays / plan / sync words must not be NULL");
    WR_REQUIRE(gs_shape_ok(user_tab, item_tab, D), WR_E_ALIGN,
               "wr_bprmf_run_sgd_group: rows must be whole 128-B lines (D %% 32 == 0, tables 128-B aligned); D = %d", (int)D);
    GroupLayout L;
    WR_REQUIRE(group_layout(n_triplets, batch_size, n_users, n_items, L), WR_E_RANGE,
               "group plan not applicable to n=%lld, batch=%lld", (long long)n_triplets, (long long)batch_size);
    WR_REQUIRE(plan_words >= L.total, WR_E_WORKSPACE, "group plan: %lld words < %lld", (long long)plan_words, (long long)L.total);
    WR_REQUIRE(first_batch >= 0 && n_batches >= 0 && first_batch + n_batches <= L.nb, WR_E_SHAPE,
               "batches [%lld,%lld) exceed the plan's %lld", (long long)first_batch, (long long)(first_batch + n_batches),
               (long long)L.nb);
    WR_REQUIRE(workspace && aligned16(workspace) && workspace_bytes >= 2 * gs_ws_one(batch_size, D), WR_E_WORKSPACE,
               "wr_bprmf_run_sgd_group: workspace %lld B < %lld B", (long long)workspace_bytes,
               (long long)(2 * gs_ws_one(batch_size, D)));
    WR_REQUIRE(aligned16(sync) && sync_words >= (n_batches + 1) * kGsStepWords + 4, WR_E_WORKSPACE,
               "wr_bprmf_run_sgd_group: %lld sync words < %lld", (long long)sync_words,
               (long long)((n_batches + 1) * kGsStepWords + 4));
    if (n_batches == 0) return WR_OK;
    static int n_cu = 0;
    if (n_cu == 0) {
        int dev = 0;
        WR_HIP(hipGetDevice(&dev));
        WR_HIP(hipDeviceGetAttribute(&n_cu, hipDeviceAttributeMultiprocessorCount, dev));
    }
    hipStream_t stream = reinterpret_cast<hipStream_t>(stream_);
    const GpDev G = group_dev(const_cast<int32_t *>(plan), L);
#define WR_CALL_GS(T_, NV_, FULL_)                                                                                          \
    return launch_group_steps<T_, NV_, FULL_>(user_tab, item_tab, D, u, p, n, n_triplets, L, G, first_batch, n_batches, lr, \
                                              loss_out, workspace, reinterpret_cast<uint32_t *>(sync), sync_words, stream,  \
                                              events, n_cu)
    WR_DISPATCH_D(D, WR_CALL_GS);
#undef WR_CALL_GS
    return WR_OK;
}

int32_t wr_bprmf_shard_step_group(float *user_shard, int64_t n_user_rows, float *item_ext, int64_t n_ext_rows,
                                  int64_t n_local_items, int32_t D, const int32_t *vu, const int32_t *vp, const int32_t *vn,
                                  int64_t n_triplets, int64_t batch_size, const int32_t *plan, int64_t plan_words, int64_t batch,
                                  int64_t global_batch, float lr, float *grad_slots, float *loss_partial, void *workspace,
                                  int64_t workspace_bytes, int32_t *sync, int64_t sync_words, void *stream_) {
    int32_t rc;
    if ((rc = check_table(user_shard, n_user_rows, D, "user_shard")) != WR_OK) return rc;
    if ((rc = check_table(item_ext, n_ext_rows, D, "item_ext")) != WR_OK) return rc;
    WR_REQUIRE(vu && vp && vn && plan && sync && grad_slots, WR_E_NULL, "index arrays / plan / sync words / grad_slots must not be NULL");
    WR_REQUIRE(aligned16(grad_slots), WR_E_ALIGN, "grad_slots is not 16-byte aligned");
    WR_REQUIRE(n_local_items >= 0 && n_local_items <= n_ext_rows, WR_E_SHAPE, "n_local_items %lld outside [0, %lld]",
               (long long)n_local_items, (long long)n_ext_rows);
    WR_REQUIRE(gs_shape_ok(user_shard, item_ext, D), WR_E_ALIGN,
               "wr_bprmf_shard_step_group: rows must be whole 128-B lines (D %% 32 == 0, tables 128-B aligned); D = %d", (int)D);
    GroupLayout L;
    WR_REQUIRE(group_layout(n_triplets, batch_size, n_user_rows, n_ext_rows, L), WR_E_RANGE,
               "group plan not applicable to n=%lld, batch=%lld", (long long)n_triplets, (long long)batch_size);
    WR_REQUIRE(plan_words >= L.total, WR_E_WORKSPACE, "group plan: %lld words < %lld", (long long)plan_words, (long long)L.total);
    WR_REQUIRE(batch >= 0 && batch < L.nb, WR_E_SHAPE, "batch %lld outside the plan's %lld", (long long)batch, (long long)L.nb);
    WR_REQUIRE(global_batch >= batch_size, WR_E_SHAPE, "global_batch %lld < local batch %lld", (long long)global_batch,
               (long long)batch_size);
    WR_REQUIRE(workspace && aligned16(workspace) && workspace_bytes >= 2 * gs_ws_one(batch_size, D), WR_E_WORKSPACE,
               "wr_bprmf_shard_step_group: workspace %lld B < %lld B", (long long)workspace_bytes,
               (long long)(2 * gs_ws_one(batch_size, D)));
    WR_REQUIRE(aligned16(sync) && sync_words >= 2 * kGsStepWords + 4, WR_E_WORKSPACE, "wr_bprmf_shard_step_group: %lld sync words < %lld",
               (long long)sync_words, (long long)(2 * kGsStepWords + 4));
    hipStream_t stream = reinterpret_cast<hipStream_t>(stream_);
    const GpDev G = group_dev(const_cast<int32_t *>(plan), L);
#define WR_CALL_GSS(T_, NV_, FULL_)                                                                                        \
    return launch_group_steps<T_, NV_, FULL_>(user_shard, item_ext, D, vu, vp, vn, n_triplets, L, G, batch, 1, lr,         \
                                              loss_partial, workspace, reinterpret_cast<uint32_t *>(sync), sync_words,     \
                                              stream, nullptr, 256, grad_slots, n_local_items, global_batch)
    WR_DISPATCH_D(D, WR_CALL_GSS);
#undef WR_CALL_GSS
    return WR_OK;
}

}
```

### whisprrec_amd/hip_ops.py

```python
import ctypes

import torch

from . import abi


def _stream():
    return torch.cuda.current_stream().cuda_stream


def _p(t):
    return None if t is None else t.data_ptr()


def _req(t, dtype, name, ndim=None):
    if not isinstance(t, torch.Tensor):
        raise TypeError("%s must be a torch.Tensor" % name)
    if t.device.type != "cuda":
        raise abi.WhisprRecHipError("%s must live on a ROCm device (got %s); there is no CPU fallback" % (name, t.device))
    if t.dtype != dtype:
        raise TypeError("%s must be %s (got %s)" % (name, dtype, t.dtype))
    if not t.is_contiguous():
        raise ValueError("%s must be contiguous" % name)
    if ndim is not None and t.dim() != ndim:
# ... 228 lines not shown
            self._unchecked = builder == "small" and not validate and not hot and not overlap
            self.meta = (torch.empty if self._unchecked else torch.zeros)(self.meta_len(self.n_batches), **i32)
            self._pinned = None
        self.torig = torch.empty(N, **i32) if keep_orig else None
        self.flags = self.meta[:2]
        self.err = self.flags[:1]
        self.hot = None
        self.builder = None
        self.overlap = None
        self.meta_host = None
        self.ready = None
        self.fast_overflowed = False
        self._finished = False
        self._sides = None
        self._tried = None
        self._backoff_key = (str(dev), self.batch_size, self.n_users, self.n_items)
        mapped = self._mapped()
        if builder == "auto" and not mapped and _FAST_BACKOFF.get(self._backoff_key, 0) > 0:
            _FAST_BACKOFF[self._backoff_key] -= 1
            builder = "generic"
            self.fast_overflowed = True
        self._builder_arg = builder
        if builder == "small":
            self._build_small()
        if builder in ("auto", "fast") and not self._build_fast():
            if builder == "fast":
                raise abi.WhisprRecHipError("fast plan builder not applicable to this batch size")
        if self._tried is None:
            self._build_generic()
        self._queue_readback()
        if not defer:
            self.finish()
            if validate:
                self.validate()

    def _mapped(self):
        bm = self._bucket_map
        return bm is not None and (bm.users is not None or bm.items is not None) and bm.batch_size == self.batch_size

    def _build_fast(self):
        L = abi.lib()
        u, p, n = self._src
        dt, dev = u.dtype, u.device
        args = (self.n_triplets, self.batch_size, self.n_users, self.n_items)
        mapped = self._mapped()
        if mapped:
            mu, mi = self._bucket_map.users, self._bucket_map.items
            nbytes = abi.check_size(L.wr_bprmf_plan_fast_mapped_workspace_bytes(*args, mu["n_buckets"] if mu else 0,
                                                                                mi["n_buckets"] if mi else 0),
                                    "wr_bprmf_plan_fast_mapped_workspace_bytes")
        else:
            nbytes = abi.check_size(L.wr_bprmf_plan_fast_workspace_bytes(*args), "wr_bprmf_plan_fast_workspace_bytes")
        if nbytes <= 0:
            return False
        ws = workspace(dev, self._ws_tag + ("_fastmap" if mapped else "_fast")).get(nbytes)
        if self._want_hot:
            self._sides = self._hot_arrays(dev)
        outs = (_p(self.tu), _p(self.tp), _p(self.tn), _p(self.torig), _p(self.oc_item), _p(self.oc_src), _p(self.flags),
                _p(ws), ws.numel(), _stream())
        self._bitmap_ready = False
        if self._want_overlap and not mapped and L.wr_bprmf_plan_fast_marks_supported(*args):
            fn = L.wr_bprmf_plan_build_fast_marks_i64 if dt == torch.int64 else L.wr_bprmf_plan_build_fast_marks_i32
            abi.check(fn(_p(u), _p(p), _p(n), *args, *outs[:-1], _p(self.arena.overlap["bitmap"]), _stream()),
                      "wr_bprmf_plan_build_fast_marks")
            self._bitmap_ready = True
        elif mapped:
            fn = L.wr_bprmf_plan_build_fast_mapped_i64 if dt == torch.int64 else L.wr_bprmf_plan_build_fast_mapped_i32
            abi.check(fn(_p(u), _p(p), _p(n), *args, ctypes.addressof(mu["struct"]) if mu else None,
                         ctypes.addressof(mi["struct"]) if mi else None, *outs), "wr_bprmf_plan_build_fast_mapped")
        else:
            fn = L.wr_bprmf_plan_build_fast_i64 if dt == torch.int64 else L.wr_bprmf_plan_build_fast_i32
            abi.check(fn(_p(u), _p(p), _p(n), *args, *outs), "wr_bprmf_plan_build_fast")
        self._tried = "fast+map" if mapped else "fast"
        if self._want_hot:
            self._enqueue_hot_runs()
        if self._want_overlap:
            self._enqueue_overlap_marks()
        return True

    def _build_small(self):
        L = abi.lib()
        u, p, n = self._src
        if self.batch_size > int(L.wr_bprmf_plan_small_max_batch()):
            raise abi.WhisprRecHipError("small plan builder: batch size %d > %d" % (self.batch_size,
                                                                                    L.wr_bprmf_plan_small_max_batch()))
        fn = L.wr_bprmf_plan_build_small_i64 if u.dtype == torch.int64 else L.wr_bprmf_plan_build_small_i32
        abi.check(fn(_p(u), _p(p), _p(n), self.n_triplets, self.batch_size, self.n_users, self.n_items, _p(self.tu), _p(self.tp),
                     _p(self.tn), _p(self.torig), _p(self.oc_item), _p(self.oc_src), None if self._unchecked else _p(self.err),
                     _stream()), "wr_bprmf_plan_build_small")
        self.builder = self._tried = "small"
        self._bitmap_ready = False
        if self._want_hot:
            self._sides = self._hot_arrays(u.device)
            self._enqueue_hot_runs()
        if self._want_overlap:
            self._enqueue_overlap_marks()

    def _build_generic(self):
        L = abi.lib()
        u, p, n = self._src
        dev = u.device
        args = (self.n_triplets, self.batch_size, self.n_users, self.n_items)
        nbytes = abi.check_size(L.wr_bprmf_plan_workspace_bytes(*args), "wr_bprmf_plan_workspace_bytes")
        ws = workspace(dev, self._ws_tag).get(nbytes)
        fn = L.wr_bprmf_plan_build_i64 if u.dtype == torch.int64 else L.wr_bprmf_plan_build_i32
        abi.check(fn(_p(u), _p(p), _p(n), *args, _p(self.tu), _p(self.tp), _p(self.tn), _p(self.torig),
                     _p(self.oc_item), _p(self.oc_src), _p(self.err), _p(ws), ws.numel(), _stream()),
                  "wr_bprmf_plan_build")
        self.builder = "generic"
        self._tried = "generic"
        self._bitmap_ready = False
        if self._want_hot:
            if self._sides is None:
                self._sides = self._hot_arrays(dev)
            self._enqueue_hot_runs()
        if self._want_overlap:
            self._enqueue_overlap_marks()

    def _hot_arrays(self, dev):
        i32 = dict(dtype=torch.int32, device=dev)
        nb = self.n_batches
        sides = []
        for kind in (0, 1):
            if self.arena is not None:
                buf, cp, cr = self.arena.hot_sides[kind]
                m = self.arena.max_batches
                arrs = [buf[:nb * cp], buf[m * cp:m * cp + nb * cp], buf[2 * m * cp:2 * m * cp + nb * cr],
                        buf[2 * m * cp + m * cr:2 * m * cp + m * cr + nb * cr],
                        buf[2 * m * cp + 2 * m * cr:2 * m * cp + 2 * m * cr + nb * cr]]
            else:
                cp, cr = hot_caps(self.batch_size, kind)
                arrs = [torch.empty(nb * cp, **i32), torch.empty(nb * cp, **i32), torch.empty(nb * cr, **i32),
                        torch.empty(nb * cr, **i32), torch.empty(nb * cr, **i32)]
            sides.append((arrs, cp, cr))
        return sides

    def _enqueue_hot_runs(self):
        L = abi.lib()
        counts = self.meta[self.META_HEAD:self.META_HEAD + 4 * self.n_batches]
        for (kind, keys), (arrs, _, _) in zip(((0, self.oc_item), (1, self.tu)), self._sides):
            abi.check(L.wr_bprmf_plan_hot_runs(_p(keys), kind, self.n_triplets, self.batch_size, *[_p(a) for a in arrs],
                                               _p(counts), _stream()), "wr_bprmf_plan_hot_runs")

    def _enqueue_overlap_marks(self):
        o, cb = self.arena.overlap, self._cap_batches
        counts = self.meta[self.META_HEAD + 4 * cb:self.META_HEAD + 5 * cb]
        L = abi.lib()
        fn = L.wr_bprmf_plan_overlap_deferred if getattr(self, "_bitmap_ready", False) else L.wr_bprmf_plan_overlap_marks
        abi.check(fn(_p(self.tu), _p(self.tp), _p(self.tn), self.n_triplets, self.batch_size, self.n_items, None,
                     _p(o["bitmap"]), _p(o["tdef"]), _p(o["def_q"]), o["cap"], _p(counts), _stream()),
                  "wr_bprmf_plan_overlap_marks")

    def _queue_readback(self):
        if self._pinned is not None:
            self._pinned.copy_(self.meta, non_blocking=True)
            self.ready = torch.cuda.Event()
            self.ready.record(self._stream)

    def _read_meta(self):
        if self._pinned is not None:
            self.ready.synchronize()
            return self._pinned
        return self.meta.cpu()

    def finish(self):
        if self._finished:
            return self
        mh = None
        while self._tried in ("fast", "fast+map") or self._want_hot:
            mh = self._read_meta()
            overflow = int(self.arena.meta_np[1]) if self._pinned is not None else int(mh[1])
            if self._tried in ("fast", "fast+map") and overflow != 0:
                if self._builder_arg == "fast":
                    raise abi.WhisprRecHipError("fast plan builder: bucket overflow (skewed ids)")
                self.fast_overflowed = True
                if self._tried == "fast":
                    _FAST_BACKOFF[self._backoff_key] = 32
                with torch.cuda.stream(self._stream):
                    self.meta.zero_()
                    self._build_generic()
                    self._queue_readback()
                mh = None
                continue
            break
        self.meta_host = mh
        if self.builder is None:
            self.builder = self._tried
        if self._want_hot:
            if self._pinned is not None:
                any_hot = bool(self.arena.meta_np[self.META_HEAD:self.META_HEAD + 4 * self.n_batches].any())
            else:
                any_hot = int(mh[self.META_HEAD:self.META_HEAD + 4 * self.n_batches].sum().item()) > 0
            if any_hot:
                self.hot = {"sides": self._sides, "counts_host": mh[self.META_HEAD:self.META_HEAD + 4 * self.n_batches]}
        if self._want_overlap and self.hot is None:
            o, nb, cb = self.arena.overlap, self.n_batches, self._cap_batches
            views = self.arena.views.get((nb, cb))
            if views is None:
                lo = self.META_HEAD + 4 * cb
                views = self.arena.views[(nb, cb)] = (mh[lo:lo + nb], self.arena.meta_np[lo:lo + nb], self.meta[lo:lo + cb])
            dc, dcn, dcd = views
            lo_n, hi_n = (int(dcn.min()), int(dcn.max())) if nb >= 2 else (-1, -1)
            if nb >= 2 and lo_n >= 0:
                self.overlap = {"tdef": o["tdef"], "def_q": o["def_q"], "def_count_host": dc, "cap": o["cap"],
                                "def_count_np": dcn, "fits": hi_n <= o["cap"], "def_count_dev": dcd}
        self._finished = True
        return self

    def hot_struct(self, batch=None):
        self.finish()
        if self.hot is None:
            return None
        k = 0 if batch is None else batch
        vals = []
        for arrs, cp, cr in self.hot["sides"]:
            vals += [arrs[0].data_ptr() + 4 * k * cp, arrs[1].data_ptr() + 4 * k * cp, arrs[2].data_ptr() + 4 * k * cr,
                     arrs[3].data_ptr() + 4 * k * cr, arrs[4].data_ptr() + 4 * k * cr]
        (_, cp0, cr0), (_, cp1, cr1) = self.hot["sides"]
        return abi.HotRuns(*vals, self.hot["counts_host"].data_ptr() + 16 * k, cp0, cr0, cp1, cr1)

    def validate(self):
        if self._unchecked:
            raise abi.WhisprRecHipError("this plan was built with validate=False and keeps no index-range flag")
        self.finish()
        if self.meta_host is None:
            self.meta_host = self._read_meta()
        bad = int(self.arena.meta_np[0]) if self._pinned is not None else int(self.meta_host[0].item())
        if bad != 0:
            raise IndexError("index out of range in batch (user_id >= n_users or item id >= n_items)")

    def batch_len(self, k):
        return min(self.batch_size, self.n_triplets - k * self.batch_size)

    def record_stream(self, stream):
        if self.arena is not None:
            return
        ts = [self.tu, self.tp, self.tn, self.oc_item, self.oc_src, self.meta]
        if self.torig is not None:
            ts.append(self.torig)
        if self._sides is not None:
            for arrs, _, _ in self._sides:
                ts += arrs
        for t in ts:
            t.record_stream(stream)


class GroupArena:

    def __init__(self, device, max_triplets, batch_size, n_users, n_items):
        words = int(abi.lib().wr_group_plan_words(int(max_triplets), int(batch_size), int(n_users), int(n_items)))
        if words <= 0:
            raise abi.WhisprRecHipError("group plan: shape not supported (batch size %d)" % batch_size)
        self.device, self.max_triplets, self.batch_size = device, int(max_triplets), int(batch_size)
        self.n_users, self.n_items = int(n_users), int(n_items)
        self.buf = torch.empty(words, dtype=torch.int32, device=device)
        self.meta_host = torch.zeros(GroupPlan.META, dtype=torch.int32, pin_memory=True)
        self.meta_np = self.meta_host.numpy()
        self.free = None

    def release_after(self, stream):
        self.free = torch.cuda.Event()
        self.free.record(stream)


class GroupPlan:

    META = 16

    def __init__(self, u, p, n, batch_size, n_users, n_items, arena=None, defer=False):
        u, p, n = (_req(t, torch.int32, nm, 1) for t, nm in ((u, "u"), (p, "p"), (n, "n")))
        N = u.numel()
        if not (p.numel() == N and n.numel() == N) or N == 0:
            raise ValueError("u/p/n must have the same non-zero length")
        L = abi.lib()
        self.u, self.p, self.n = u, p, n
        self.n_triplets, self.batch_size = N, int(batch_size)
        self.n_users, self.n_items = int(n_users), int(n_items)
        self.n_batches = (N + self.batch_size - 1) // self.batch_size
        self.words = int(L.wr_group_plan_words(N, self.batch_size, self.n_users, self.n_items))
        if self.words <= 0:
            raise abi.WhisprRecHipError("group plan: shape not supported (batch size %d)" % self.batch_size)
        self.arena = arena
        self._stream = torch.cuda.current_stream(u.device)
        if arena is not None:
            if arena.buf.numel() < self.words or arena.batch_size != self.batch_size or \
                    (arena.n_users, arena.n_items) != (self.n_users, self.n_items):
                raise ValueError("plan does not fit its arena")
            if arena.free is not None:
                self._stream.wait_event(arena.free)
                arena.free = None
            self.buf = arena.buf
            self._pinned = arena.meta_host
        else:
            self.buf = torch.empty(self.words, dtype=torch.int32, device=u.device)
            self._pinned = None
        abi.check(L.wr_group_plan_build(_p(u), _p(p), _p(n), N, self.batch_size, self.n_users, self.n_items, _p(self.buf),
                                        self.buf.numel(), _stream()), "wr_group_plan_build")
        self.ready = None
        if self._pinned is not None:
            self._pinned.copy_(self.buf[:self.META], non_blocking=True)
            self.ready = torch.cuda.Event()
            self.ready.record(self._stream)
        self._finished = False
        self.bad_index = self.overflow = self.long_run = False
        if not defer:
            self.finish()

    def finish(self):
        if self._finished:
            return self
        if self._pinned is not None:
            self.ready.synchronize()
            m = self.arena.meta_np
        else:
            m = self.buf[:self.META].cpu().numpy()
        self.bad_index, self.overflow, self.long_run = bool(m[0]), bool(m[1]), bool(m[2])
        self._finished = True
        return self

    def finish_from(self, meta):
        self.bad_index, self.overflow, self.long_run = bool(meta[0]), bool(meta[1]), bool(meta[2])
        self._finished = True
        return self

    def validate(self):
        self.finish()
        if self.bad_index:
            raise IndexError("index out of range in batch (user_id >= n_users or item id >= n_items)")

    def batch_len(self, k):
        return min(self.batch_size, self.n_triplets - k * self.batch_size)

    def layout(self):
        out = (ctypes.c_int64 * 16)()
        abi.check(abi.lib().wr_group_plan_layout(self.n_triplets, self.batch_size, self.n_users, self.n_items,
                                                 ctypes.addressof(out)), "wr_group_plan_layout")
        keys = ("nb", "fw", "R_u", "R_i", "mask_u", "mask_i", "flags", "ucnt", "icnt", "ul_row", "ul_src", "il_row", "il_src",
                "total", "cap_u", "cap_i")
        return dict(zip(keys, [int(v) for v in out]))

    def decode(self):
        import numpy as np
        self.finish()
        Ly = self.layout()
        w = self.buf[:Ly["total"]].cpu().numpy()
        nb, fw = Ly["nb"], Ly["fw"]
        flags = w[Ly["flags"]:Ly["flags"] + nb * fw * 4].view(np.uint32).reshape(nb, fw, 4).copy()
        out = {"flags": flags, "users": {}, "items": {}, "R_u": Ly["R_u"], "R_i": Ly["R_i"], "meta": w[:self.META].copy()}
        for side, R, cap, co, ro, so in (("users", Ly["R_u"], Ly["cap_u"], "ucnt", "ul_row", "ul_src"),
                                         ("items", Ly["R_i"], Ly["cap_i"], "icnt", "il_row", "il_src")):
            for b in range(nb):
                for r in range(R):
                    c = int(w[Ly[co] + b * R + r])
                    at = (b * R + r) * cap
                    out[side][(b, r)] = (w[Ly[ro] + at:Ly[ro] + at + c].astype(np.int64),
                                         w[Ly[so] + at:Ly[so] + at + c].astype(np.int64))
        return out


_CHAIN_SYNC = {}
_OVERLAP_WS_BYTES = {}


class BprmfTables:

    def __init__(self, user_tab, item_tab):
        self.U = _req(user_tab, torch.float32, "user_tab", 2)
        self.I = _req(item_tab, torch.float32, "item_tab", 2)
        if self.U.shape[1] != self.I.shape[1]:
            raise ValueError("user and item tables must have the same embedding size")
        self.D = self.U.shape[1]
        self.dev = self.U.device
        self.stamp_u = None
        self.stamp_i = None
        self.step_id = 0

    def _stamps(self):
        if self.stamp_u is None:
            self.stamp_u = torch.full((self.U.shape[0],), -1, dtype=torch.int32, device=self.dev)
            self.stamp_i = torch.full((self.I.shape[0],), -1, dtype=torch.int32, device=self.dev)
        return self.stamp_u, self.stamp_i

    def _ws(self, B):
        nbytes = abi.check_size(abi.lib().wr_bprmf_step_workspace_bytes(B, self.D), "wr_bprmf_step_workspace_bytes")
        return workspace(self.dev, "step").get(nbytes)

    def _plan_ptrs(self, plan, k):
        off = k * plan.batch_size
        return (plan.tu.data_ptr() + 4 * off, plan.tp.data_ptr() + 4 * off, plan.tn.data_ptr() + 4 * off,
                plan.oc_item.data_ptr() + 8 * off, plan.oc_src.data_ptr() + 8 * off, plan.batch_len(k))

    def step_sgd(self, plan, k, lr, l2=0.0, loss_out=None, decay_untouched=True):
        L = abi.lib()
        tu, tp, tn, oi, os_, B = self._plan_ptrs(plan, k)
        ws = self._ws(plan.batch_size)
        if loss_out is None:
            loss_out = torch.empty((), dtype=torch.float32, device=self.dev)
        su = si = None
        self.step_id += 1
        if l2 != 0.0:
            su, si = self._stamps()
        hot = plan.hot_struct(k)
        abi.check(L.wr_bprmf_step_sgd(_p(self.U), self.U.shape[0], _p(self.I), self.I.shape[0], self.D, tu, tp, tn, oi,
                                      os_, B, lr, l2, _p(su), _p(si), self.step_id, _p(loss_out),
                                      ctypes.addressof(hot) if hot is not None else None, _p(ws), ws.numel(),
                                      _stream()), "wr_bprmf_step_sgd")
        if l2 != 0.0 and decay_untouched:
            abi.check(L.wr_sgd_decay_untouched(_p(self.U), self.U.shape[0], self.D, _p(su), self.step_id, lr, l2,
                                               _stream()), "wr_sgd_decay_untouched")
            abi.check(L.wr_sgd_decay_untouched(_p(self.I), self.I.shape[0], self.D, _p(si), self.step_id, lr, l2,
                                               _stream()), "wr_sgd_decay_untouched")
        return loss_out

    def run_sgd(self, plan, first, count, lr, losses=None, phase_events=None):
        L = abi.lib()
        ws = self._ws(plan.batch_size)
        if losses is None:
            losses = torch.empty(count, dtype=torch.float32, device=self.dev)
        hot = plan.hot_struct()
        ev = None
        if phase_events is not None:
            if len(phase_events) != 4 * count:
                raise ValueError("phase_events must hold 4 events per step")
            handles = []
            for e in phase_events:
                if e is None:
                    handles.append(None)
                    continue
                if not e.cuda_event:
                    e.record()
                handles.append(e.cuda_event)
            ev = (ctypes.c_void_p * len(handles))(*handles)
        abi.check(L.wr_bprmf_run_sgd(_p(self.U), self.U.shape[0], _p(self.I), self.I.shape[0], self.D, _p(plan.tu),
                                     _p(plan.tp), _p(plan.tn), _p(plan.oc_item), _p(plan.oc_src), plan.n_triplets,
                                     plan.batch_size, first, count, lr, _p(losses),
                                     ctypes.addressof(ev) if ev is not None else None,
                                     ctypes.addressof(hot) if hot is not None else None, _p(ws), ws.numel(), _stream()),
                  "wr_bprmf_run_sgd")
        self.step_id += count
        return losses

    def overlap_workspace(self, batch_size):
        nbytes = _OVERLAP_WS_BYTES.get((batch_size, self.D))
        if nbytes is None:
            nbytes = _OVERLAP_WS_BYTES[(batch_size, self.D)] = 2 * abi.check_size(
                abi.lib().wr_bprmf_step_workspace_bytes(batch_size, self.D), "wr_bprmf_step_workspace_bytes")
        return workspace(self.dev, "step_overlap").get(nbytes)

    def chain_supported(self):
        return bool(abi.lib().wr_bprmf_chain_supported(_p(self.U), _p(self.I), self.D))

    CHAIN_SYNC_STEPS = 256

    def _chain_sync(self, count):
        key = (str(self.dev), torch.cuda.current_stream(self.dev).cuda_stream)
        bufs = _CHAIN_SYNC.setdefault(key, [])
        if bufs and count <= self.CHAIN_SYNC_STEPS:
            return bufs[-1]
        if not bufs or bufs[-1].numel() < int(abi.lib().wr_bprmf_chain_sync_words(count)):
            words = int(abi.lib().wr_bprmf_chain_sync_words(max(count, self.CHAIN_SYNC_STEPS)))
            bufs.append(torch.zeros(words, dtype=torch.int32, device=self.dev))
        return bufs[-1]

    def sticky_words(self):
        sid = torch.cuda.current_stream(self.dev).cuda_stream
        return [buf[-4:-3] for key, bufs in _CHAIN_SYNC.items() if key[0] == str(self.dev) and key[1] == sid for buf in bufs]

    def check_chain(self):
        for key, bufs in _CHAIN_SYNC.items():
            if key[0] != str(self.dev):
                continue
            for buf in bufs:
                if int(buf[-4].item()) != 0:
                    raise abi.WhisprRecHipError("chained step launch: a wait for the item tiles expired — the tables are "
                                                "not valid")

    def run_sgd_chain(self, plan, first, count, lr, losses=None, phase_events=None, ws=None, def_limit=None):
        L = abi.lib()
        o = plan.overlap
        if ws is None:
            ws = self.overlap_workspace(plan.batch_size)
        if losses is None:
            losses = torch.empty(count, dtype=torch.float32, device=self.dev)
        ev = None
        if phase_events is not None:
            if len(phase_events) != 4 * count:
                raise ValueError("phase_events must hold 4 events per step")
            handles = []
            for e in phase_events:
                if e is None:
                    handles.append(None)
                    continue
                if not e.cuda_event:
                    e.record()
                handles.append(e.cuda_event)
            ev = (ctypes.c_void_p * len(handles))(*handles)
        sync = self._chain_sync(count)
        abi.check(L.wr_bprmf_run_sgd_chain(_p(self.U), self.U.shape[0], _p(self.I), self.I.shape[0], self.D, _p(plan.tu),
                                           _p(plan.tp), _p(plan.tn), _p(plan.oc_item), _p(plan.oc_src), plan.n_triplets,
                                           plan.batch_size, first, count, lr, _p(losses), _p(o["tdef"]), _p(o["def_q"]),
                                           o["def_count_host"].data_ptr(), o["cap"],
                                           o["cap"] if def_limit is None else int(def_limit),
                                           ctypes.addressof(ev) if ev is not None else None, _p(ws), ws.numel(), _p(sync),
                                           sync.numel(), _stream()), "wr_bprmf_run_sgd_chain")
        self.step_id += count
        return losses

    def group_supported(self):
        return bool(abi.lib().wr_bprmf_group_supported(_p(self.U), _p(self.I), self.D))

    def _group_sync(self, count):
        key = (str(self.dev), torch.cuda.current_stream(self.dev).cuda_stream, "group")
        bufs = _CHAIN_SYNC.setdefault(key, [])
        need = int(abi.lib().wr_bprmf_group_sync_words(count))
        if not bufs or bufs[-1].numel() < need:
            words = int(abi.lib().wr_bprmf_group_sync_words(max(count, self.CHAIN_SYNC_STEPS)))
            bufs.append(torch.zeros(words, dtype=torch.int32, device=self.dev))
        return bufs[-1]

    def run_sgd_group(self, gplan, first, count, lr, losses=None, events=None):
        L = abi.lib()
        nbytes = abi.check_size(L.wr_bprmf_group_workspace_bytes(gplan.batch_size, self.D), "wr_bprmf_group_workspace_bytes")
        ws = workspace(self.dev, "group_step").get(nbytes)
        if losses is None:
            losses = torch.empty(count, dtype=torch.float32, device=self.dev)
        ev = None
        if events is not None:
            if len(events) != 2 * count:
                raise ValueError("events must hold 2 events per step")
            handles = []
            for e in events:
                if not e.cuda_event:
                    e.record()
                handles.append(e.cuda_event)
            ev = (ctypes.c_void_p * len(handles))(*handles)
        sync = self._group_sync(count)
        abi.check(L.wr_bprmf_run_sgd_group(_p(self.U), self.U.shape[0], _p(self.I), self.I.shape[0], self.D, _p(gplan.u),
                                           _p(gplan.p), _p(gplan.n), gplan.n_triplets, gplan.batch_size, _p(gplan.buf),
                                           gplan.buf.numel(), first, count, lr, _p(losses),
                                           ctypes.addressof(ev) if ev is not None else None, _p(ws), ws.numel(), _p(sync),
                                           sync.numel(), _stream()), "wr_bprmf_run_sgd_group")
        self.step_id += count
        return losses

    def grads(self, plan, k, grad_u, grad_i, loss_out=None, stamps=True):
        L = abi.lib()
        tu, tp, tn, oi, os_, B = self._plan_ptrs(plan, k)
        ws = self._ws(plan.batch_size)
        su, si = self._stamps() if stamps else (None, None)
        if loss_out is None:
            loss_out = torch.empty((), dtype=torch.float32, device=self.dev)
        self.step_id += 1
        hot = plan.hot_struct(k)
        abi.check(L.wr_bprmf_grads(_p(self.U), self.U.shape[0], _p(self.I), self.I.shape[0], self.D, tu, tp, tn, oi, os_,
                                   B, _p(grad_u), _p(grad_i), _p(su), _p(si), self.step_id, _p(loss_out),
                                   ctypes.addressof(hot) if hot is not None else None, _p(ws), ws.numel(), _stream()),
                  "wr_bprmf_grads")
        return loss_out, self.step_id


PAIR_SET_MIN_PAIRS = 1 << 20


def pair_set(clicked_ptr, clicked_idx, n_users):
    _req(clicked_ptr, torch.int64, "clicked_ptr", 1)
    _req(clicked_idx, torch.int32, "clicked_idx", 1)
    L = abi.lib()
    cap = abi.check_size(L.wr_pairset_capacity(int(clicked_idx.numel())), "wr_pairset_capacity")
    table = torch.empty(cap, dtype=torch.int64, device=clicked_ptr.device)
    err = torch.zeros(1, dtype=torch.int32, device=clicked_ptr.device)
    abi.check(L.wr_pairset_build(_p(clicked_ptr), _p(clicked_idx), int(n_users), _p(table), cap, _p(err), _stream()),
              "wr_pairset_build")
    if int(err.item()) != 0:
        raise abi.WhisprRecHipError("pair set: table too small")
    return table


def sample_negatives(users, n_users, n_items, clicked_ptr, clicked_idx, seed, epoch, pairs=None):
    if users.dtype not in (torch.int64, torch.int32):
        raise TypeError("users must be int64 or int32")
    users = _req(users.contiguous(), users.dtype, "users", 1)
    if pairs is None:
        _req(clicked_ptr, torch.int64, "clicked_ptr", 1)
        _req(clicked_idx, torch.int32, "clicked_idx", 1)
    neg = torch.empty_like(users)
    err = torch.zeros(1, dtype=torch.int32, device=users.device)
    L = abi.lib()
    if pairs is not None:
        fn = L.wr_sample_negatives_set_i64 if users.dtype == torch.int64 else L.wr_sample_negatives_set_i32
        abi.check(fn(_p(users), users.numel(), n_users, n_items, _p(_req(pairs, torch.int64, "pairs", 1)), pairs.numel(), seed,
                     epoch, _p(neg), _p(err), _stream()), "wr_sample_negatives_set")
        return neg, err
    fn = L.wr_sample_negatives_i64 if users.dtype == torch.int64 else L.wr_sample_negatives_i32
    abi.check(fn(_p(users), users.numel(), n_users, n_items, _p(clicked_ptr), _p(clicked_idx), seed, epoch, _p(neg), _p(err),
                 _stream()), "wr_sample_negatives")
    return neg, err


def epoch_shuffle(cols, seed, epoch, want_order=False):
    cols = list(cols)
    if not 1 <= len(cols) <= 3:
        raise ValueError("one to three columns")
    dt = cols[0].dtype
    if dt not in (torch.int64, torch.int32):
        raise TypeError("columns must be int64 or int32")
    n = cols[0].numel()
    cols = [_req(c.contiguous(), dt, "column", 1) for c in cols]
    if any(c.numel() != n for c in cols):
        raise ValueError("columns must have the same length")
    outs = [torch.empty_like(c) for c in cols]
    order = torch.empty(n, dtype=torch.int64, device=cols[0].device) if want_order else None
    pad = [None] * (3 - len(cols))
    fn = abi.lib().wr_epoch_shuffle_i64 if dt == torch.int64 else abi.lib().wr_epoch_shuffle_i32
    abi.check(fn(*[_p(c) for c in cols + pad], n, int(seed), int(epoch), *[_p(o) for o in outs + pad], _p(order), _stream()),
              "wr_epoch_shuffle")
    return (outs, order) if want_order else outs


class EpochPrep:

    def __init__(self, users, items, n_users, n_items, clicked_ptr, clicked_idx, seed, epoch, want_order=False, pairs=None,
                 packed=None):
        if users.dtype not in (torch.int64, torch.int32) or items.dtype != users.dtype:
            raise TypeError("users / items must both be int64 or int32")
        self.users = _req(users.contiguous(), users.dtype, "users", 1)
        self.items = _req(items.contiguous(), users.dtype, "items", 1)
        if self.items.numel() != self.users.numel():
            raise ValueError("users / items must have the same length")
        if pairs is None:
            _req(clicked_ptr, torch.int64, "clicked_ptr", 1)
            _req(clicked_idx, torch.int32, "clicked_idx", 1)
        self.ptr, self.idx = clicked_ptr, clicked_idx
        self.pairs = None if pairs is None else _req(pairs, torch.int64, "pairs", 1)
        self.packed = None
        if packed is not None and pairs is not None:
            self.packed = _req(packed, torch.int64, "packed", 1)
            if self.packed.numel() != self.users.numel():
                raise ValueError("packed rows: one word per interaction")
        self.n, self.n_users, self.n_items = users.numel(), int(n_users), int(n_items)
        self.seed, self.epoch = int(seed), int(epoch)
        self.cols = [torch.empty_like(self.users) for _ in range(3)]
        self.order = torch.empty(self.n, dtype=torch.int64, device=users.device) if want_order else None
        self.err = torch.zeros(1, dtype=torch.int32, device=users.device)
        self.filled = 0

    def fill(self, lo, hi):
        lo, hi = int(lo), min(int(hi), self.n)
        if hi <= lo:
            return
        es = self.users.element_size()
        L = abi.lib()
        tail = (self.seed, self.epoch, lo, hi - lo, self.cols[0].data_ptr() + es * lo, self.cols[1].data_ptr() + es * lo,
                self.cols[2].data_ptr() + es * lo, None if self.order is None else self.order.data_ptr() + 8 * lo,
                _p(self.err), _stream())
        if self.packed is not None:
            fn = L.wr_epoch_prepare_range_packed_i64 if self.users.dtype == torch.int64 else L.wr_epoch_prepare_range_packed_i32
            abi.check(fn(_p(self.packed), self.n, self.n_users, self.n_items, _p(self.pairs), self.pairs.numel(), *tail),
                      "wr_epoch_prepare_range_packed")
        elif self.pairs is not None:
            fn = L.wr_epoch_prepare_range_set_i64 if self.users.dtype == torch.int64 else L.wr_epoch_prepare_range_set_i32
            abi.check(fn(_p(self.users), _p(self.items), self.n, self.n_users, self.n_items, _p(self.pairs), self.pairs.numel(),
                         *tail), "wr_epoch_prepare_range_set")
        else:
            fn = L.wr_epoch_prepare_range_i64 if self.users.dtype == torch.int64 else L.wr_epoch_prepare_range_i32
            abi.check(fn(_p(self.users), _p(self.items), self.n, self.n_users, self.n_items, _p(self.ptr), _p(self.idx), *tail),
                      "wr_epoch_prepare_range")
        self.filled = max(self.filled, hi)

    def check(self):
        if int(self.err.item()) == 1:
            raise IndexError("user id out of range in the training frame")


def pack_rows(users, items):
    return ((users.to(torch.int64) << 32) | items.to(torch.int64)).contiguous()


def clicked_csr_from_pairs(users, items, n_users, n_items):
    key = torch.unique(users.to(torch.int64) * int(n_items) + items.to(torch.int64))
    uu = torch.div(key, int(n_items), rounding_mode="floor")
    ptr = torch.zeros(n_users + 1, dtype=torch.int64, device=users.device)
    ptr[1:] = torch.cumsum(torch.bincount(uu, minlength=n_users), 0)
    return ptr, (key - uu * int(n_items)).to(torch.int32)


def clicked_csr(train_clicked_set, n_users, device):
    import numpy as np
    ptr = np.zeros(n_users + 1, np.int64)
    chunks = []
    for uu in range(n_users):
        items = train_clicked_set.get(uu, ())
        ptr[uu + 1] = ptr[uu] + len(items)
        if len(items):
            chunks.append(np.sort(np.fromiter(items, dtype=np.int32, count=len(items))))
    idx = np.concatenate(chunks) if chunks else np.zeros(1, np.int32)
    return torch.from_numpy(ptr).to(device), torch.from_numpy(idx).to(device)


LDS_PER_WORKGROUP = 160 * 1024


def rank_eval_supports(D):
    D = int(D)
    if D % 4 != 0 or D < 4:
        return False
    return D in (8, 16, 32, 64) or ((128 + 32) * (D + 1) + 128) * 4 <= LDS_PER_WORKGROUP


def rank_eval(user_mat, item_tab, eval_user, eval_target, mask_ptr=None, mask_idx=None):
    _req(user_mat, torch.float32, "user_mat", 2)
    _req(item_tab, torch.float32, "item_tab", 2)
    eu, et = _idx64(eval_user.reshape(-1), "eval_user"), _idx64(eval_target.reshape(-1), "eval_target")
    if mask_ptr is not None:
        _req(mask_ptr, torch.int64, "mask_ptr", 1)
        _req(mask_idx, torch.int32, "mask_idx", 1)
    n = eu.numel()
    rank = torch.empty(n, dtype=torch.int32, device=user_mat.device)
    tsc = torch.empty(n, dtype=torch.float32, device=user_mat.device)
    abi.check(abi.lib().wr_rank_eval(_p(user_mat), user_mat.shape[0], _p(item_tab), item_tab.shape[0], user_mat.shape[1],
                                     _p(eu), _p(et), n, _p(mask_ptr), _p(mask_idx), _p(rank), _p(tsc), _stream()),
              "wr_rank_eval")
    return rank, tsc


TOPK_MAX_K = 256
TOPK_WORKSPACE_CAP = 2 << 30


def topk_supports(D, k):
    return bool(abi.lib().wr_topk_supported(int(D), int(k)))


def topk_recommend(user_mat, item_tab, users, k, mask_ptr=None, mask_idx=None):
    _req(user_mat, torch.float32, "user_mat", 2)
    _req(item_tab, torch.float32, "item_tab", 2)
    qu = _idx64(users.reshape(-1), "users")
    if (mask_ptr is None) != (mask_idx is None):
        raise ValueError("mask_ptr and mask_idx go together")
    if mask_ptr is not None:
        _req(mask_ptr, torch.int64, "mask_ptr", 1)
        _req(mask_idx, torch.int32, "mask_idx", 1)
    k, D = int(k), int(user_mat.shape[1])
    if item_tab.shape[1] != D:
        raise ValueError("user_mat and item_tab have different widths (%d, %d)" % (D, item_tab.shape[1]))
    if not topk_supports(D, k):
        raise abi.WhisprRecHipError("topk_recommend does not support D=%d, k=%d (1 <= k <= %d; D as for rank_eval)"
                                    % (D, k, TOPK_MAX_K))
    L, dev = abi.lib(), user_mat.device
    n, n_items = qu.numel(), item_tab.shape[0]
    items = torch.empty((n, k), dtype=torch.int32, device=dev)
    scores = torch.empty((n, k), dtype=torch.float32, device=dev)
    block = max(n, 1)
    while block > 128 and abi.check_size(L.wr_topk_workspace_bytes(block, n_items, D, k), "wr_topk_workspace_bytes") \
            > TOPK_WORKSPACE_CAP:
        block = (block + 1) // 2
    ws = workspace(dev, "topk")
    for lo in range(0, n, block):
        hi = min(n, lo + block)
        nb = abi.check_size(L.wr_topk_workspace_bytes(hi - lo, n_items, D, k), "wr_topk_workspace_bytes")
        buf = ws.get(nb)
        abi.check(L.wr_topk_recommend(_p(user_mat), user_mat.shape[0], _p(item_tab), n_items, D, _p(qu[lo:hi]), hi - lo,
                                      _p(mask_ptr), _p(mask_idx), k, _p(items[lo:hi]), _p(scores[lo:hi]), _p(buf),
                                      buf.numel(), _stream()),
                  "wr_topk_recommend")
    return items.to(torch.int64), scores


def sgd_dense(tab, grad, lr, l2=0.0, stamp=None, step_id=0):
    abi.check(abi.lib().wr_sgd_dense(_p(_req(tab, torch.float32, "tab", 2)), tab.shape[0], tab.shape[1],
                                     _p(_req(grad, torch.float32, "grad", 2)), _p(stamp), step_id, lr, l2, _stream()),
              "wr_sgd_dense")


def adam_dense(tab, exp_avg, exp_avg_sq, grad, adam_step, lr, l2=0.0, beta1=0.9, beta2=0.999, eps=1e-8, stamp=None,
               step_id=0):
    for t, nm in ((tab, "tab"), (exp_avg, "exp_avg"), (exp_avg_sq, "exp_avg_sq"), (grad, "grad")):
        _req(t, torch.float32, nm, 2)
    abi.check(abi.lib().wr_adam_dense(_p(tab), _p(exp_avg), _p(exp_avg_sq), tab.shape[0], tab.shape[1], _p(grad),
                                      _p(stamp), step_id, adam_step, lr, l2, beta1, beta2, eps, _stream()),
              "wr_adam_dense")


def _join_views(ts):
    if len(ts) == 1:
        return ts[0]
    a = ts[0]
    adjacent, end = a.is_contiguous(), a.storage_offset() + a.numel()
    for b in ts[1:]:
        adjacent = adjacent and b.is_contiguous() and b.dtype == a.dtype and \
            b.untyped_storage().data_ptr() == a.untyped_storage().data_ptr() and b.storage_offset() == end
        end += b.numel()
    if adjacent:
        return torch.as_strided(a, (end - a.storage_offset(),), (1,), a.storage_offset())
    return torch.cat(ts)


class PipelinedSgd:

    PREFETCH_AFTER_TRIPLETS = 0
    PLAN_TRIPLETS = 1 << 22
    GROUP_MIN_ROWS_PER_TRIPLET = 12
    GROUP_MIN_BATCH = 4096

    CHAIN_MIN_BATCH = 8192
    CHAIN_MIN_ITEMS_PER_TRIPLET = 6

    def __init__(self, chunk=64, min_triplets=None, chain=True, inline_plan=False, group=True):
        import sys
        self.ops = sys.modules[__name__]
        self.chunk = int(chunk)
        self.chain = bool(chain)
        self.group = bool(group)
        self.inline_plan = inline_plan
        self.stats = {"plain_calls": 0, "chain_calls": 0, "group_calls": 0, "group_fallbacks": 0}
        self._garenas = {}
        if min_triplets is not None:
            self.PLAN_TRIPLETS = int(min_triplets)
        self.plan_stream = None
        self._arenas = {}

    def chunk_batches(self, batch_size):
        return max(self.chunk, self.PLAN_TRIPLETS // max(int(batch_size), 1))

    def _arena_pair(self, device, B, nb_total, overlap_items):
        cap = min(self.chunk_batches(B), max(int(nb_total), 1)) * B
        key = (str(device), B, int(overlap_items))
        pair = self._arenas.get(key)
        if pair is None or pair[0].max_triplets < cap:
            pair = [self.ops.PlanArena(device, cap, B, overlap_items=overlap_items) for _ in range(2)]
            self._arenas[key] = pair
        return pair

    def _garena_pair(self, device, B, nb_total, n_users, n_items):
        cap = min(self.chunk_batches(B), max(int(nb_total), 1)) * B
        key = (str(device), B, int(n_users), int(n_items))
        pair = self._garenas.get(key)
        if pair is None or pair[0].max_triplets < cap:
            pair = [self.ops.GroupArena(device, cap, B, n_users, n_items) for _ in range(2)]
            self._garenas[key] = pair
        return pair

    def plan(self, U, segments, batch, first_chunk=None, lr=None, prep=None, runner=None):
        if self.plan_stream is None:
            self.plan_stream = side_stream(U.device)
# ... 714 lines not shown
```

Measured before the change: 2.749 billion triplets/s.

## Group shared-row triplets into connected components and update each component in one team block

Adds a plan-build kernel that runs union-find over triplets sharing user/item rows within each batch. It packs small components (up to 16 triplets) into slots so one block can apply their conflicting updates together via LDS exchange, and marks large components for the old path. The step kernel gains a component route that replaces chained/serialized handling of shared rows, and the Python side picks it unless the plan flags oversize. This adds plan-build work and an extra finish() sync on the host before each step launch, and it is risky if the fallback is taken for many batches.

```diff
diff --git a/include/whisprrec_hip.h b/include/whisprrec_hip.h
--- a/include/whisprrec_hip.h
+++ b/include/whisprrec_hip.h
@@ -169,6 +169,7 @@
 
 int64_t wr_group_plan_words(int64_t n_triplets, int64_t batch_size, int64_t n_users, int64_t n_items);
 int32_t wr_group_plan_layout(int64_t n_triplets, int64_t batch_size, int64_t n_users, int64_t n_items, int64_t *out);
+int32_t wr_group_plan_comp_layout(int64_t n_triplets, int64_t batch_size, int64_t n_users, int64_t n_items, int64_t *out);
 int32_t wr_narrow_ids_i64(const int64_t *u, const int64_t *p, const int64_t *n, int32_t *u32, int32_t *p32, int32_t *n32,
                           int64_t count, void *stream);
 int32_t wr_group_plan_build(const int32_t *u, const int32_t *p, const int32_t *n, int64_t n_triplets, int64_t batch_size,
@@ -180,7 +181,7 @@
                                const int32_t *u, const int32_t *p, const int32_t *n, int64_t n_triplets, int64_t batch_size,
                                const int32_t *plan, int64_t plan_words, int64_t first_batch, int64_t n_batches, float lr,
                                float *loss_out, void *const *events, void *workspace, int64_t workspace_bytes, int32_t *sync,
-                               int64_t sync_words, void *stream);
+                               int64_t sync_words, int32_t components, void *stream);
 
 int32_t wr_bprmf_plan_overlap_marks(const int32_t *tu, const int32_t *tp, const int32_t *tn, int64_t n_triplets,
                                     int64_t batch_size, int64_t n_items, const int32_t *prev_bitmap, int32_t *bitmap,
diff --git a/whisprrec_amd/abi.py b/whisprrec_amd/abi.py
--- a/whisprrec_amd/abi.py
+++ b/whisprrec_amd/abi.py
@@ -79,13 +79,14 @@
                                           c_i64, c_i64, c_f32, c_vp, c_vp, c_vp, c_i64, c_vp, c_i64, c_vp]),
     "wr_group_plan_words": (c_i64, [c_i64, c_i64, c_i64, c_i64]),
     "wr_group_plan_layout": (c_i32, [c_i64, c_i64, c_i64, c_i64, c_vp]),
+    "wr_group_plan_comp_layout": (c_i32, [c_i64, c_i64, c_i64, c_i64, c_vp]),
     "wr_narrow_ids_i64": (c_i32, [c_vp, c_vp, c_vp, c_vp, c_vp, c_vp, c_i64, c_vp]),
     "wr_group_plan_build": (c_i32, [c_vp, c_vp, c_vp, c_i64, c_i64, c_i64, c_i64, c_vp, c_i64, c_vp]),
     "wr_bprmf_group_workspace_bytes": (c_i64, [c_i64, c_i32]),
     "wr_bprmf_group_sync_words": (c_i64, [c_i64]),
     "wr_bprmf_group_supported": (c_i32, [c_vp, c_vp, c_i32]),
     "wr_bprmf_run_sgd_group": (c_i32, [c_vp, c_i64, c_vp, c_i64, c_i32, c_vp, c_vp, c_vp, c_i64, c_i64, c_vp, c_i64, c_i64,
-                                       c_i64, c_f32, c_vp, c_vp, c_vp, c_i64, c_vp, c_i64, c_vp]),
+                                       c_i64, c_f32, c_vp, c_vp, c_vp, c_i64, c_vp, c_i64, c_i32, c_vp]),
     "wr_bprmf_plan_overlap_deferred": (c_i32, [c_vp, c_vp, c_vp, c_i64, c_i64, c_i64, c_vp, c_vp, c_vp, c_vp, c_i64, c_vp,
                                                c_vp]),
     "wr_bprmf_plan_fast_marks_supported": (c_i32, [c_i64, c_i64, c_i64, c_i64]),
diff --git a/whisprrec_amd/csrc/wr_group.hip b/whisprrec_amd/csrc/wr_group.hip
--- a/whisprrec_amd/csrc/wr_group.hip
+++ b/whisprrec_amd/csrc/wr_group.hip
@@ -25,6 +25,7 @@
     unsigned mask_u, mask_i, hbits_u, hbits_i;
     int64_t flags, ucnt, icnt, ul_row, ul_src, il_row, il_src, total;
     int64_t zero_words;
+    int64_t ctri, cslot, cmark, ct_stride, cs_stride, cm_stride;
 };
 
 static inline int ranges_for(int64_t n_rows, unsigned *mask, unsigned *hbits, int *cap) {
@@ -53,7 +54,13 @@
     L.ul_src = L.ul_row + L.nb * L.R_u * (int64_t)L.cap_u;
     L.il_row = L.ul_src + L.nb * L.R_u * (int64_t)L.cap_u;
     L.il_src = L.il_row + L.nb * L.R_i * (int64_t)L.cap_i;
-    L.total = L.il_src + L.nb * L.R_i * (int64_t)L.cap_i;
+    L.ct_stride = align_up(B, 4);
+    L.cs_stride = align_up(B + 2, 4);
+    L.cm_stride = align_up(L.fw, 4);
+    L.ctri = L.il_src + L.nb * L.R_i * (int64_t)L.cap_i;
+    L.cslot = L.ctri + L.nb * L.ct_stride;
+    L.cmark = L.cslot + L.nb * L.cs_stride;
+    L.total = L.cmark + L.nb * L.cm_stride;
     return true;
 }
 
@@ -65,12 +72,17 @@
     int R_u, R_i, cap_u, cap_i;
     unsigned mask_u, mask_i, hbits_u, hbits_i;
     int fw;
+    int *ctri;
+    int *cslot;
+    unsigned *cmark;
+    int ct_stride, cs_stride, cm_stride;
 };
 
 static inline GpDev group_dev(int32_t *plan, const GroupLayout &L) {
     return GpDev{plan, reinterpret_cast<unsigned *>(plan + L.flags), plan + L.ucnt, plan + L.icnt, plan + L.ul_row,
                  plan + L.ul_src, plan + L.il_row, plan + L.il_src, L.R_u, L.R_i, L.cap_u, L.cap_i, L.mask_u, L.mask_i,
-                 L.hbits_u, L.hbits_i, (int)L.fw};
+                 L.hbits_u, L.hbits_i, (int)L.fw, plan + L.ctri, plan + L.cslot, reinterpret_cast<unsigned *>(plan + L.cmark),
+                 (int)L.ct_stride, (int)L.cs_stride, (int)L.cm_stride};
 }
 
 template <typename F>
@@ -271,6 +283,222 @@
     if (threadIdx.x == 0) (item ? L.icnt : L.ucnt)[(int64_t)b * R + r] = m;
 }
 
+constexpr int kCompTeams = 16;
+constexpr int kCompMaxLinked = 24576;
+constexpr int kCompLanes = 64;
+
+__device__ __forceinline__ int gc_load(const int *a) { return __hip_atomic_load(a, __ATOMIC_RELAXED, __HIP_MEMORY_SCOPE_WORKGROUP); }
+
+__device__ __forceinline__ int gc_find(int *par, int x) {
+    for (;;) {
+        const int p = gc_load(par + x);
+        if (p == x) return x;
+        const int gp = gc_load(par + p);
+        if (gp != p) __hip_atomic_store(par + x, gp, __ATOMIC_RELAXED, __HIP_MEMORY_SCOPE_WORKGROUP);
+        x = gp;
+    }
+}
+
+__device__ __forceinline__ void gc_unite(int *par, int a, int b) {
+    for (;;) {
+        a = gc_find(par, a);
+        b = gc_find(par, b);
+        if (a == b) return;
+        if (a > b) {
+            const int x = a;
+            a = b;
+            b = x;
+        }
+        if (atomicCAS(par + b, b, a) == b) return;
+    }
+}
+
+__device__ __forceinline__ int gc_scan(int v, int *wt, int &total) {
+    int incl = v;
+#pragma unroll
+    for (int d = 1; d < 64; d <<= 1) {
+        const int x = __shfl_up(incl, d, 64);
+        if ((int)(threadIdx.x & 63) >= d) incl += x;
+    }
+    const int wave = (int)threadIdx.x >> 6;
+    if ((threadIdx.x & 63) == 63) wt[wave] = incl;
+    __syncthreads();
+    int before = 0, tot = 0;
+#pragma unroll
+    for (int w = 0; w < kGpThreads / 64; ++w) {
+        const int x = wt[w];
+        before += w < wave ? x : 0;
+        tot += x;
+    }
+    total = tot;
+    __syncthreads();
+    return before + incl - v;
+}
+
+__global__ __launch_bounds__(kGpThreads) void group_comp_kernel(int64_t n_total, int B, GpDev L) {
+    extern __shared__ __attribute__((aligned(16))) unsigned gc_lds[];
+    const int fw = L.fw;
+    unsigned *link = gc_lds;
+    int *wpre = reinterpret_cast<int *>(link + fw);
+    int *misc = wpre + fw;
+    int *par = misc + 32;
+    const int b = (int)blockIdx.x;
+    const uint4 *fl = reinterpret_cast<const uint4 *>(L.flags) + (int64_t)b * fw;
+    int *ctri = L.ctri + (int64_t)b * L.ct_stride, *cslot = L.cslot + (int64_t)b * L.cs_stride;
+    unsigned *cmark = L.cmark + (int64_t)b * L.cm_stride;
+    (void)n_total;
+    const int per_w = (fw + kGpThreads - 1) / kGpThreads, w0 = (int)threadIdx.x * per_w;
+    int mine = 0;
+    for (int w = w0; w < min(fw, w0 + per_w); ++w) {
+        const uint4 f = fl[w];
+        const unsigned m = f.x | f.y | f.z;
+        link[w] = m;
+        mine += __popc(m);
+        cmark[w] = 0u;
+    }
+    int n_linked;
+    int before = gc_scan(mine, misc, n_linked);
+    for (int w = w0; w < min(fw, w0 + per_w); ++w) {
+        wpre[w] = before;
+        before += __popc(link[w]);
+    }
+    if (n_linked > kCompMaxLinked) {
+        for (int w = threadIdx.x; w < fw; w += kGpThreads) cmark[w] = link[w];
+        if (threadIdx.x == 0) {
+            cslot[0] = 0;
+            cslot[1] = 0;
+            L.meta[3] = 1;
+        }
+        return;
+    }
+    for (int i = threadIdx.x; i < n_linked; i += kGpThreads) par[i] = i;
+    __syncthreads();
+    auto idx = [&](int t) -> int {
+        const int w = t >> 5;
+        return wpre[w] + __popc(link[w] & ((1u << (t & 31)) - 1u));
+    };
+    auto linked = [&](int t) -> bool { return t >= 0 && (t >> 5) < fw && ((link[t >> 5] >> (t & 31)) & 1u); };
+    for (int side = 0; side < 2; ++side) {
+        const int R = side ? L.R_i : L.R_u, cap = side ? L.cap_i : L.cap_u;
+        const int *cnt = (side ? L.icnt : L.ucnt) + (int64_t)b * R;
+        for (int seg = 0; seg < R; ++seg) {
+            const int m = min(cnt[seg], cap);
+            const int *rows = (side ? L.il_row : L.ul_row) + ((int64_t)b * R + seg) * cap;
+            const int *src = (side ? L.il_src : L.ul_src) + ((int64_t)b * R + seg) * cap;
+            for (int e = (int)threadIdx.x + 1; e < m; e += kGpThreads) {
+                if (rows[e] != rows[e - 1]) continue;
+                const int ta = src[e] >> 1, tb = src[e - 1] >> 1;
+                if (linked(ta) && linked(tb)) gc_unite(par, idx(ta), idx(tb));
+            }
+        }
+    }
+    __syncthreads();
+    for (int i = threadIdx.x; i < n_linked; i += kGpThreads) {
+        const int r = gc_find(par, i);
+        if (r != i) __hip_atomic_store(par + i, r, __ATOMIC_RELAXED, __HIP_MEMORY_SCOPE_WORKGROUP);
+    }
+    __syncthreads();
+    for (int i = threadIdx.x; i < n_linked; i += kGpThreads) atomicAdd(par + (gc_load(par + i) & 0xFFFF), 1 << 16);
+    __syncthreads();
+    const int per = (n_linked + kGpThreads - 1) / kGpThreads, i0 = (int)threadIdx.x * per, i1 = min(n_linked, i0 + per);
+    int sum = 0;
+    for (int i = i0; i < i1; ++i) {
+        const int v = par[i];
+        const int sz = v >> 16;
+        if ((v & 0xFFFF) == i && sz <= kCompTeams) sum += sz;
+    }
+    int n_slotted;
+    int at = gc_scan(sum, misc, n_slotted);
+    bool big = false;
+    for (int i = i0; i < i1; ++i) {
+        const int v = par[i];
+        if ((v & 0xFFFF) != i) continue;
+        const int sz = v >> 16;
+        if (sz <= kCompTeams) {
+            par[i] = (int)(0x80000000u | ((unsigned)sz << 15) | (unsigned)at);
+            at += sz;
+        } else {
+            par[i] = (int)(0x40000000u | ((unsigned)sz << 15));
+            big = true;
+        }
+    }
+    if (big) L.meta[3] = 1;
+    __syncthreads();
+    for (int w = threadIdx.x; w < fw; w += kGpThreads) {
+        unsigned m = link[w];
+        if (!m) continue;
+        const uint4 f = fl[w];
+        int i = wpre[w];
+        unsigned mk = 0u;
+        while (m) {
+            const int bit = __ffs(m) - 1;
+            m &= m - 1;
+            const int v = gc_load(par + i);
+            const int r = (v >> 30) == 0 ? v : i;
+            const unsigned rw = (unsigned)(r == i ? v : gc_load(par + r));
+            if (rw & 0x40000000u) {
+                mk |= 1u << bit;
+            } else {
+                const int slot = (atomicAdd(par + r, 1) & 0x7FFF);
+                ctri[slot] = ((w * 32 + bit) << 3) | (int)((((f.x >> bit) & 1u) << 2) | (((f.z >> bit) & 1u) << 1) | ((f.y >> bit) & 1u));
+            }
+            ++i;
+        }
+        if (mk) cmark[w] = mk;
+    }
+    __syncthreads();
+    for (int i = i0; i < i1; ++i) {
+        const unsigned v = (unsigned)par[i];
+        if (!(v & 0x80000000u)) continue;
+        const int sz = (int)((v >> 15) & 0x7FFFu), end = (int)(v & 0x7FFFu), st = end - sz;
+        for (int j = st + 1; j < end; ++j) {
+            const int x = ctri[j];
+            int k = j - 1;
+            while (k >= st && ctri[k] > x) {
+                ctri[k + 1] = ctri[k];
+                --k;
+            }
+            ctri[k + 1] = x;
+        }
+    }
+    if (threadIdx.x < 64) {
+        const int C = (n_linked + kCompLanes - 1) / kCompLanes, k0 = (int)threadIdx.x * C, k1 = min(n_linked, k0 + C);
+        int ns = 0, fill = kCompTeams + 1;
+        for (int i = k0; i < k1; ++i) {
+            const unsigned v = (unsigned)par[i];
+            if (!(v & 0x80000000u)) continue;
+            const int sz = (int)((v >> 15) & 0x7FFFu);
+            if (fill + sz > kCompTeams) {
+                ++ns;
+                fill = 0;
+            }
+            fill += sz;
+        }
+        int incl = ns;
+#pragma unroll
+        for (int d = 1; d < 64; d <<= 1) {
+            const int x = __shfl_up(incl, d, 64);
+            if ((int)threadIdx.x >= d) incl += x;
+        }
+        int s = incl - ns;
+        fill = kCompTeams + 1;
+        for (int i = k0; i < k1; ++i) {
+            const unsigned v = (unsigned)par[i];
+            if (!(v & 0x80000000u)) continue;
+            const int sz = (int)((v >> 15) & 0x7FFFu);
+            if (fill + sz > kCompTeams) {
+                cslot[1 + s++] = (int)(v & 0x7FFFu) - sz;
+                fill = 0;
+            }
+            fill += sz;
+        }
+        if (threadIdx.x == 63) {
+            cslot[0] = incl;
+            cslot[1 + incl] = n_slotted;
+        }
+    }
+}
+
 __global__ __launch_bounds__(kBlock) void narrow_ids_kernel(const int64_t *__restrict__ u, const int64_t *__restrict__ p,
                                                              const int64_t *__restrict__ n, int *__restrict__ u32,
                                                              int *__restrict__ p32, int *__restrict__ n32, int64_t cnt) {
@@ -296,6 +524,7 @@
     const uint4 *flags;
     const int *ul_row, *ul_src, *ul_cnt, *il_row, *il_src, *il_cnt;
     int B, R_u, R_i, cap_u, cap_i;
+    const int *ctri, *cslot;
 };
 
 struct GsArgs {
@@ -315,6 +544,8 @@
     unsigned *done, *timeout;
     float *Gs;
     int nL;
+    int comp, nC, fold;
+    const int *meta;
 };
 
 template <int NV>
@@ -382,6 +613,126 @@
         }
     }
     if (ps || ns) store_row<T, NV, FULL>(a.Z, t, a.D, lane, z);
+}
+
+template <int T, int NV, bool FULL>
+__device__ __forceinline__ void gs_components(const GsArgs &a, int w, int lane, float &terms, float4 *__restrict__ xg,
+                                              int4 *__restrict__ xid) {
+    const int team = (int)threadIdx.x / T;
+    const int n_slots = a.cur.cslot[0];
+    const float lr = a.lr;
+    for (int s = w; s < n_slots; s += a.nC) {
+        const int o0 = a.cur.cslot[1 + s], o1 = a.cur.cslot[2 + s];
+        const int cnt = min(o1 - o0, kCompTeams);
+        const bool act = team < cnt;
+        int e = 0, t = 0, u = 0, p = 0, n = 0;
+        if (act) {
+            e = a.cur.ctri[o0 + team];
+            t = min(max(e >> 3, 0), a.cur.B - 1);
+            u = a.cur.u[t];
+            p = a.cur.p[t];
+            n = a.cur.n[t];
+        }
+        const bool us = e & 4, ns = e & 2, ps = e & 1;
+        Row<NV> ur = row_zero<NV>(), pr = row_zero<NV>(), nr = row_zero<NV>(), g, z;
+        float c = 0.f;
+        if (act) {
+            ur = load_row<T, NV, FULL>(a.U, u, a.D, lane);
+            pr = load_row<T, NV, FULL>(a.I, p, a.D, lane);
+            nr = load_row<T, NV, FULL>(a.I, n, a.D, lane);
+        }
+        const float sp = team_sum<T>(dot_partial<NV>(ur, pr));
+        const float sn = team_sum<T>(dot_partial<NV>(ur, nr));
+        if (act) {
+            float term;
+            bpr_terms(sp, sn, a.denom, term, c);
+            terms += term;
+        }
+#pragma unroll
+        for (int k = 0; k < NV; ++k) {
+            g.v[k] = make_float4(c * (pr.v[k].x - nr.v[k].x), c * (pr.v[k].y - nr.v[k].y), c * (pr.v[k].z - nr.v[k].z),
+                                 c * (pr.v[k].w - nr.v[k].w));
+            z.v[k] = make_float4(c * ur.v[k].x, c * ur.v[k].y, c * ur.v[k].z, c * ur.v[k].w);
+        }
+        if (team < kCompTeams) {
+#pragma unroll
+            for (int k = 0; k < NV; ++k) {
+                xg[((team * 2 + 0) * NV + k) * T + lane] = g.v[k];
+                xg[((team * 2 + 1) * NV + k) * T + lane] = z.v[k];
+            }
+            if (lane == 0) xid[team] = act ? make_int4(u, p, n, 0) : make_int4(-1, -1, -1, 0);
+        }
+        __syncthreads();
+        if (act) {
+            auto add = [&](Row<NV> &acc, int i, int kind, float sgn) {
+#pragma unroll
+                for (int k = 0; k < NV; ++k) {
+                    const float4 x = xg[((i * 2 + kind) * NV + k) * T + lane];
+                    acc.v[k].x = fmaf(sgn, x.x, acc.v[k].x);
+                    acc.v[k].y = fmaf(sgn, x.y, acc.v[k].y);
+                    acc.v[k].z = fmaf(sgn, x.z, acc.v[k].z);
+                    acc.v[k].w = fmaf(sgn, x.w, acc.v[k].w);
+                }
+            };
+            auto finish = [&](float *W, int row, const Row<NV> &r0, const Row<NV> &acc) {
+                Row<NV> wv;
+#pragma unroll
+                for (int k = 0; k < NV; ++k)
+                    wv.v[k] = make_float4(r0.v[k].x - lr * acc.v[k].x, r0.v[k].y - lr * acc.v[k].y, r0.v[k].z - lr * acc.v[k].z,
+                                          r0.v[k].w - lr * acc.v[k].w);
+                store_row<T, NV, FULL>(W, row, a.D, lane, wv);
+            };
+            if (!us) {
+                finish(a.U, u, ur, g);
+            } else {
+                bool first = true;
+                for (int i = 0; i < team; ++i) first = first && xid[i].x != u;
+                if (first) {
+                    Row<NV> acc = row_zero<NV>();
+                    add(acc, team, 0, 1.0f);
+                    for (int i = team + 1; i < cnt; ++i)
+                        if (xid[i].x == u) add(acc, i, 0, 1.0f);
+                    finish(a.U, u, ur, acc);
+                }
+            }
+            auto item_sum = [&](int row, float s0, const Row<NV> &r0) {
+                Row<NV> acc = row_zero<NV>();
+                add(acc, team, 1, s0);
+                if (s0 > 0.f && n == row) add(acc, team, 1, -1.0f);
+                for (int i = team + 1; i < cnt; ++i) {
+                    const int4 x = xid[i];
+                    if (x.y == row) add(acc, i, 1, 1.0f);
+                    if (x.z == row) add(acc, i, 1, -1.0f);
+                }
+                finish(a.I, row, r0, acc);
+            };
+            auto earlier = [&](int row) {
+                bool seen = false;
+                for (int i = 0; i < team; ++i) {
+                    const int4 x = xid[i];
+                    seen = seen || x.y == row || x.z == row;
+                }
+                return seen;
+            };
+            if (!ps) {
+                Row<NV> zp = z;
+                finish(a.I, p, pr, zp);
+            } else if (!earlier(p)) {
+                item_sum(p, 1.0f, pr);
+            }
+            if (!ns) {
+                Row<NV> w;
+#pragma unroll
+                for (int k = 0; k < NV; ++k)
+                    w.v[k] = make_float4(nr.v[k].x - lr * (-z.v[k].x), nr.v[k].y - lr * (-z.v[k].y), nr.v[k].z - lr * (-z.v[k].z),
+                                         nr.v[k].w - lr * (-z.v[k].w));
+                store_row<T, NV, FULL>(a.I, n, a.D, lane, w);
+            } else if (p != n && !earlier(n)) {
+                item_sum(n, -1.0f, nr);
+            }
+        }
+        __syncthreads();
+    }
 }
 
 __device__ __forceinline__ void gs_wait_tiles(const GsArgs &a) {
@@ -557,11 +908,37 @@
 
 template <int T, int NV, bool FULL>
 __global__ __launch_bounds__(kBlock, NV == 1 ? WR_GS_WAVES : 1) void bprmf_group_step(GsArgs a) {
+    constexpr int kXg = NV <= 2 ? kCompTeams * 2 * T * NV : 0;
+    constexpr int kLdsInts = kGsLdsInts > 4 * (kXg + kCompTeams) ? kGsLdsInts : 4 * (kXg + kCompTeams);
     __shared__ float scratch[kBlock / 64];
-    __shared__ __attribute__((aligned(16))) int lds[kGsLdsInts];
+    __shared__ __attribute__((aligned(16))) int lds[kLdsInts];
     constexpr int TEAMS = kBlock / T;
     const int lane = threadIdx.x % T;
     int b = (int)blockIdx.x;
+    if (a.comp) {
+        if (b >= a.nC + a.nA) {
+            if (a.loss_prev != nullptr) {
+                const float s0 = strided_partial_sum(a.partials_prev, a.n_partials_prev);
+                const float s = block_sum(s0, scratch);
+                if (threadIdx.x == 0) a.loss_prev[0] = s / a.denom_prev;
+            }
+            return;
+        }
+        if (b < a.nC) {
+            float terms = 0.f;
+            if constexpr (NV <= 2) {
+                if (b == 0 && threadIdx.x == 0 && a.meta[3] != 0)
+                    __hip_atomic_store(a.timeout, 2u, __ATOMIC_RELAXED, __HIP_MEMORY_SCOPE_AGENT);
+                gs_components<T, NV, FULL>(a, b, lane, terms, reinterpret_cast<float4 *>(lds),
+                                           reinterpret_cast<int4 *>(lds) + kXg);
+            }
+            if (lane != 0) terms = 0.f;
+            const float sum = block_sum(terms, scratch);
+            if (threadIdx.x == 0) a.partials[a.nA + b] = sum;
+            return;
+        }
+        b -= a.nC;
+    }
     if (b >= a.tiles_at && b < a.tiles_at + a.nIT + a.nUT) {
         const int w = b - a.tiles_at;
         const bool wt = a.nA > 0;
@@ -665,7 +1042,7 @@
 #endif
         asm volatile("" : "+v"(u), "+v"(p), "+v"(n), "+v"(f.x), "+v"(f.y), "+v"(f.z), "+v"(f.w));
         const unsigned bit = 1u << (t & 31);
-        if (t < a.cur.B && !(a.chained && (f.w & bit)))
+        if (t < a.cur.B && !(a.chained && (f.w & bit)) && !(a.comp && ((f.x | f.y | f.z) & bit)))
             gs_single<T, NV, FULL>(a, t, u, p, n, f.x & bit, f.y & bit, f.z & bit, lane, terms);
         slot = b;
     }
@@ -676,9 +1053,13 @@
 
 static inline int gs_teams_per_block(int D) { return D >= 64 ? kBlock / 16 : (D == 32 ? kBlock / 8 : (D == 16 ? kBlock / 4 : (D == 8 ? kBlock / 2 : (D == 4 ? kBlock : kBlock / 16)))); }
 
+#ifndef WR_GS_NC_DIV
+#define WR_GS_NC_DIV 48
+#endif
+
 static inline int64_t gs_ws_one(int64_t B, int32_t D) {
     const int64_t nA = (B + gs_teams_per_block(D) - 1) / gs_teams_per_block(D);
-    return 2 * align_up(B * (int64_t)D * 4, 256) + align_up((nA + 512) * 4, 256);
+    return 2 * align_up(B * (int64_t)D * 4, 256) + align_up((nA + 512 + B / WR_GS_NC_DIV + 1) * 4, 256);
 }
 
 static inline bool gs_shape_ok(const float *U, const float *I, int32_t D) {
@@ -706,7 +1087,8 @@
                                   int64_t n_triplets, const GroupLayout &L, const GpDev &G, int64_t first_batch,
                                   int64_t n_batches, float lr, float *loss_out, void *workspace, uint32_t *sync,
                                   int64_t sync_words, hipStream_t stream, void *const *events, int n_cu,
-                                  float *grad_slots = nullptr, int64_t n_local_items = 0, int64_t global_batch = 0) {
+                                  float *grad_slots = nullptr, int64_t n_local_items = 0, int64_t global_batch = 0,
+                                  int components = 0) {
     const int64_t B = L.B;
     const int64_t ws_one = gs_ws_one(B, D), zb = align_up(B * (int64_t)D * 4, 256);
     char *ws = reinterpret_cast<char *>(workspace);
@@ -714,7 +1096,8 @@
     float *ZUs[2] = {reinterpret_cast<float *>(ws + zb), reinterpret_cast<float *>(ws + ws_one + zb)};
     float *Ps[2] = {reinterpret_cast<float *>(ws + 2 * zb), reinterpret_cast<float *>(ws + ws_one + 2 * zb)};
     constexpr int TEAMS = kBlock / T;
-    WR_HIP(hipMemsetAsync(sync, 0, (size_t)(n_batches * kGsStepWords) * 4, stream));
+    const bool comp = components != 0 && NV <= 2 && grad_slots == nullptr;
+    if (!comp) WR_HIP(hipMemsetAsync(sync, 0, (size_t)(n_batches * kGsStepWords) * 4, stream));
     uint32_t *timeout = sync + (sync_words - 4);
     int nDS = WR_GS_NDS;
     while (nDS > n_cu / 4 && nDS > 1) nDS >>= 1;
@@ -724,10 +1107,46 @@
         return GsBatch{u + off, p + off, n + off, reinterpret_cast<const uint4 *>(G.flags + b * L.fw * 4),
                        G.ul_row + b * L.R_u * (int64_t)L.cap_u, G.ul_src + b * L.R_u * (int64_t)L.cap_u, G.ucnt + b * L.R_u,
                        G.il_row + b * L.R_i * (int64_t)L.cap_i, G.il_src + b * L.R_i * (int64_t)L.cap_i, G.icnt + b * L.R_i,
-                       Bk, L.R_u, L.R_i, L.cap_u, L.cap_i};
+                       Bk, L.R_u, L.R_i, L.cap_u, L.cap_i, G.ctri + b * (int64_t)G.ct_stride, G.cslot + b * (int64_t)G.cs_stride};
     };
     auto ev = [&](int64_t k, int j) { return events ? reinterpret_cast<hipEvent_t>(events[2 * k + j]) : (hipEvent_t) nullptr; };
     int n_partials_prev = 0;
+    if (comp) {
+        for (int64_t k = 0; k <= n_batches; ++k) {
+            if (k == n_batches && loss_out == nullptr) break;
+            GsArgs a{};
+            a.U = U;
+            a.I = I;
+            a.D = D;
+            a.lr = lr;
+            a.timeout = timeout;
+            a.comp = 1;
+            a.meta = G.meta;
+            if (k < n_batches) {
+                a.cur = batch_of(first_batch + k);
+                a.partials = Ps[k & 1];
+                a.denom = (float)a.cur.B;
+                a.nA = (int)((a.cur.B + TEAMS - 1) / TEAMS);
+                a.nC = (int)std::max<int64_t>(1, (B + WR_GS_NC_DIV - 1) / WR_GS_NC_DIV);
+            }
+            if (k > 0) {
+                a.fold = 1;
+                a.partials_prev = Ps[(k - 1) & 1];
+                a.n_partials_prev = n_partials_prev;
+                a.denom_prev = (float)batch_of(first_batch + k - 1).B;
+                a.loss_prev = loss_out ? loss_out + (k - 1) : nullptr;
+            }
+            const dim3 grid((unsigned)(a.nC + a.nA + a.fold));
+            hipEvent_t e0 = k < n_batches ? ev(k, 0) : nullptr, e1 = k < n_batches ? ev(k, 1) : nullptr;
+            if (e0 != nullptr || e1 != nullptr)
+                hipExtLaunchKernelGGL((bprmf_group_step<T, NV, FULL>), grid, dim3(kBlock), 0, stream, e0, e1, 0, a);
+            else
+                hipLaunchKernelGGL((bprmf_group_step<T, NV, FULL>), grid, dim3(kBlock), 0, stream, a);
+            WR_LAUNCH_CHECK("bprmf_group_step");
+            n_partials_prev = a.nA + a.nC;
+        }
+        return WR_OK;
+    }
     for (int64_t k = 0; k <= n_batches; ++k) {
         GsArgs a{};
         a.U = U;
@@ -797,6 +1216,16 @@
     return WR_OK;
 }
 
+int32_t wr_group_plan_comp_layout(int64_t n_triplets, int64_t batch_size, int64_t n_users, int64_t n_items, int64_t *out) {
+    WR_REQUIRE(out != nullptr, WR_E_NULL, "out is NULL");
+    GroupLayout L;
+    WR_REQUIRE(group_layout(n_triplets, batch_size, n_users, n_items, L), WR_E_RANGE,
+               "group plan not applicable to n=%lld, batch=%lld", (long long)n_triplets, (long long)batch_size);
+    const int64_t v[8] = {L.ctri, L.ct_stride, L.cslot, L.cs_stride, L.cmark, L.cm_stride, kCompTeams, kCompMaxLinked};
+    for (int i = 0; i < 8; ++i) out[i] = v[i];
+    return WR_OK;
+}
+
 int32_t wr_narrow_ids_i64(const int64_t *u, const int64_t *p, const int64_t *n, int32_t *u32, int32_t *p32, int32_t *n32,
                           int64_t count, void *stream_) {
     WR_REQUIRE(u && p && n && u32 && p32 && n32, WR_E_NULL, "index arrays must not be NULL");
@@ -830,6 +1259,15 @@
     hipLaunchKernelGGL(group_plan_kernel, dim3((unsigned)(L.nb * (L.R_u + L.R_i))), dim3(kGpThreads), lds, stream, u, p, n,
                        n_triplets, (int)batch_size, (int)L.nb, (int)n_users, (int)n_items, G);
     WR_LAUNCH_CHECK("group_plan_kernel");
+    const size_t lds_c = (size_t)(2 * L.fw + 32 + kCompMaxLinked) * 4;
+    static bool attr_c = false;
+    if (!attr_c) {
+        WR_HIP(hipFuncSetAttribute(reinterpret_cast<const void *>(group_comp_kernel), hipFuncAttributeMaxDynamicSharedMemorySize,
+                                   (int)((2 * ((kGpMaxBatch + 31) / 32) + 32 + kCompMaxLinked) * 4)));
+        attr_c = true;
+    }
+    hipLaunchKernelGGL(group_comp_kernel, dim3((unsigned)L.nb), dim3(kGpThreads), lds_c, stream, n_triplets, (int)batch_size, G);
+    WR_LAUNCH_CHECK("group_comp_kernel");
     return WR_OK;
 }
 
@@ -845,7 +1283,7 @@
                                const int32_t *u, const int32_t *p, const int32_t *n, int64_t n_triplets, int64_t batch_size,
                                const int32_t *plan, int64_t plan_words, int64_t first_batch, int64_t n_batches, float lr,
                                float *loss_out, void *const *events, void *workspace, int64_t workspace_bytes, int32_t *sync,
-                               int64_t sync_words, void *stream_) {
+                               int64_t sync_words, int32_t components, void *stream_) {
     int32_t rc;
     if ((rc = check_table(user_tab, n_users, D, "user_tab")) != WR_OK) return rc;
     if ((rc = check_table(item_tab, n_items, D, "item_tab")) != WR_OK) return rc;
@@ -877,7 +1315,7 @@
 #define WR_CALL_GS(T_, NV_, FULL_)                                                                                          \
     return launch_group_steps<T_, NV_, FULL_>(user_tab, item_tab, D, u, p, n, n_triplets, L, G, first_batch, n_batches, lr, \
                                               loss_out, workspace, reinterpret_cast<uint32_t *>(sync), sync_words, stream,  \
-                                              events, n_cu)
+                                              events, n_cu, nullptr, 0, 0, components)
     WR_DISPATCH_D(D, WR_CALL_GS);
 #undef WR_CALL_GS
     return WR_OK;
diff --git a/whisprrec_amd/hip_ops.py b/whisprrec_amd/hip_ops.py
--- a/whisprrec_amd/hip_ops.py
+++ b/whisprrec_amd/hip_ops.py
@@ -554,7 +554,7 @@
             self.ready = torch.cuda.Event()
             self.ready.record(self._stream)
         self._finished = False
-        self.bad_index = self.overflow = self.long_run = False
+        self.bad_index = self.overflow = self.long_run = self.oversize = False
         if not defer:
             self.finish()
 
@@ -567,11 +567,13 @@
         else:
             m = self.buf[:self.META].cpu().numpy()
         self.bad_index, self.overflow, self.long_run = bool(m[0]), bool(m[1]), bool(m[2])
+        self.oversize = bool(m[3])
         self._finished = True
         return self
 
     def finish_from(self, meta):
         self.bad_index, self.overflow, self.long_run = bool(meta[0]), bool(meta[1]), bool(meta[2])
+        self.oversize = True
         self._finished = True
         return self
 
@@ -590,6 +592,28 @@
         keys = ("nb", "fw", "R_u", "R_i", "mask_u", "mask_i", "flags", "ucnt", "icnt", "ul_row", "ul_src", "il_row", "il_src",
                 "total", "cap_u", "cap_i")
         return dict(zip(keys, [int(v) for v in out]))
+
+    def comp_layout(self):
+        out = (ctypes.c_int64 * 8)()
+        abi.check(abi.lib().wr_group_plan_comp_layout(self.n_triplets, self.batch_size, self.n_users, self.n_items,
+                                                      ctypes.addressof(out)), "wr_group_plan_comp_layout")
+        keys = ("ctri", "ct_stride", "cslot", "cs_stride", "cmark", "cm_stride", "comp_teams", "max_linked")
+        return dict(zip(keys, [int(v) for v in out]))
+
+    def decode_components(self):
+        import numpy as np
+        self.finish()
+        C = self.comp_layout()
+        w = self.buf.cpu().numpy()
+        out = []
+        for b in range(self.n_batches):
+            cs = w[C["cslot"] + b * C["cs_stride"]:C["cslot"] + (b + 1) * C["cs_stride"]]
+            ns = int(cs[0])
+            slots = cs[1:ns + 2].astype(np.int64)
+            tri = w[C["ctri"] + b * C["ct_stride"]:C["ctri"] + b * C["ct_stride"] + int(slots[-1])].astype(np.int64)
+            mark = w[C["cmark"] + b * C["cm_stride"]:C["cmark"] + b * C["cm_stride"] + (self.batch_size + 31) // 32]
+            out.append((tri, slots, mark.view(np.uint32).copy()))
+        return out
 
     def decode(self):
         import numpy as np
@@ -770,8 +794,10 @@
             bufs.append(torch.zeros(words, dtype=torch.int32, device=self.dev))
         return bufs[-1]
 
-    def run_sgd_group(self, gplan, first, count, lr, losses=None, events=None):
+    def run_sgd_group(self, gplan, first, count, lr, losses=None, events=None, old_route=False):
         L = abi.lib()
+        gplan.finish()
+        components = 0 if (old_route or gplan.oversize) else 1
         nbytes = abi.check_size(L.wr_bprmf_group_workspace_bytes(gplan.batch_size, self.D), "wr_bprmf_group_workspace_bytes")
         ws = workspace(self.dev, "group_step").get(nbytes)
         if losses is None:
@@ -791,7 +817,7 @@
                                            _p(gplan.p), _p(gplan.n), gplan.n_triplets, gplan.batch_size, _p(gplan.buf),
                                            gplan.buf.numel(), first, count, lr, _p(losses),
                                            ctypes.addressof(ev) if ev is not None else None, _p(ws), ws.numel(), _p(sync),
-                                           sync.numel(), _stream()), "wr_bprmf_run_sgd_group")
+                                           sync.numel(), components, _stream()), "wr_bprmf_run_sgd_group")
         self.step_id += count
         return losses
 
```

New measurement: 2.694 billion triplets/s (median of 2 runs). -2.0%, worse.
